# AleoNet/snarkVM

Measured on AMD Instinct MI355X. Metric: BLS12-377 G1 MSM scalar-point pairs/sec (+ Fr NTT elements/sec in ntt_*), higher is better.
Workload: dtype u32 limbs (29-bit radix) modular integer arithmetic, Fq 377-bit / Fr 253-bit; 1 GPU; G1 Pippenger MSM 2^24 (BASELINE.json configs[1]), bases (i+1)G registered in HBM, uniform scalars in HBM; independent instance per GPU; scalars=uniform, lg_ntt=24, window_bits=auto, base_tables=12, table_bits=22, pipelined_batch=True

## Files before the change

### snarkvm_amd/csrc/api_g2.hip

```cpp
#include "msm_batch.hip.h"
#include "serde.hip.h"

static void tu_set_kernel_attributes() {
    HIP_TRY(hipFuncSetAttribute((const void*)scan_one_block_kernel, hipFuncAttributeMaxDynamicSharedMemorySize, (int)(SCAN_ONE_MAX * 4)));
}

struct snarkvm_hip_bases_g2 : bases_handle_t<fq2_t> {};

extern "C" {

RustError snarkvm_hip_msm_g2(void* out, const void* points, size_t npoints, const void* scalars, size_t ffi_affine_sz) {
    API_TRY
#ifdef SV_NO_G2
    throw hip_failure{hipErrorNotSupported, "this development build was compiled without G2 (SV_NO_G2)", __LINE__};
#else
    if (!out) throw hip_failure{hipErrorInvalidValue, "msm_g2: null output", __LINE__};
    g_rt.configure();
    if (npoints == 0) {
        write_infinity<fq2_t>(out);
    } else {
        if (!points || !scalars) throw hip_failure{hipErrorInvalidValue, "msm_g2: null argument", __LINE__};
        msm_host_chunked<fq2_t>(out, points, npoints, scalars, ffi_affine_sz);
    }
#endif
    API_CATCH
}

RustError snarkvm_hip_register_bases_g2(snarkvm_hip_bases_g2_t** handle, const void* points, size_t npoints, size_t ffi_affine_sz, int tables,
                                        int window_bits) {
    API_TRY
#ifdef SV_NO_G2
    throw hip_failure{hipErrorNotSupported, "this development build was compiled without G2 (SV_NO_G2)", __LINE__};
#else
    if (!handle || (npoints && !points)) throw hip_failure{hipErrorInvalidValue, "register_bases_g2: null argument", __LINE__};
    if (ffi_affine_sz < 200 || (ffi_affine_sz & 7)) throw hip_failure{hipErrorInvalidValue, "register_bases_g2: bad stride", __LINE__};
    check_tables(tables, window_bits, "register_bases_g2");
    const int nd = g_rt.ndev();
    std::unique_ptr<snarkvm_hip_bases_g2> h(new snarkvm_hip_bases_g2());
    h->n = npoints;
    h->tables = tables;
    h->table_bits = window_bits ? window_bits : 256 / tables;
    h->d.assign(nd, nullptr);
    if (npoints) {
        try {
            std::vector<int> all;
            for (int d = 0; d < nd; d++) all.push_back(d);
            for_each_device(all, [&](int dev) {
                lane_guard lg(dev);
                lane_t& c = lg.c();
                HIP_TRY(hipMalloc((void**)&h->d[dev], (size_t)tables * npoints * sizeof(aff_mem_t<fq2_t>)));
                c.bases_tmp.ensure(npoints * ffi_affine_sz);
                HIP_TRY(hipMemcpyAsync(c.bases_tmp.p, points, npoints * ffi_affine_sz, hipMemcpyHostToDevice, c.stream));
                convert_bases<fq2_t>(c, c.bases_tmp.as<uint8_t>(), ffi_affine_sz, npoints, h->d[dev]);
                precompute_tables_run<fq2_t>(c, h->d[dev], npoints, tables, h->table_bits);
                bases_to_lazy_form(c, h->d[dev], (size_t)tables * npoints);
                HIP_TRY(hipStreamSynchronize(c.stream));
            });
        } catch (...) {
            h->free_all();
            throw;
        }
    }
    *handle = h.release();
#endif
    API_CATCH
}
void snarkvm_hip_free_bases_g2(snarkvm_hip_bases_g2_t* h) {
    if (!h) return;
    h->free_all();
    delete h;
}
#ifndef SV_NO_G2
static RustError msm_g2_single_coalesced(void* out, const snarkvm_hip_bases_g2_t* h, size_t offset, size_t npoints, const void* scalars, int scalars_on_device,
                                         int window_bits) {
    API_TRY
    if (scalars_on_device && g_rt.device_of(scalars) < 0)
        throw hip_failure{hipErrorInvalidValue, "device pointer does not belong to a device in use (snarkvm_hip_set_devices)", __LINE__};
    msm_ticket_t t;
    t.req.off0 = offset, t.req.n0 = npoints, t.req.scalars = scalars, t.req.out = out;
    t.on_device = scalars_on_device ? 1 : 0;
    t.window_bits = window_bits;
    msm_coalesced<fq2_t>(*h, &t, 1);
    API_CATCH
}
static RustError msm_g2_scope_enqueue(void* out, const snarkvm_hip_bases_g2_t* h, size_t offset, size_t npoints, const void* scalars, int window_bits, bool* queued) {
    API_TRY
    msm_req_t one;
    one.off0 = offset, one.n0 = npoints, one.scalars = scalars, one.out = out;
    *queued = msm_scope_enqueue<fq2_t>(*h, &one, 1, 1, 0, window_bits);
    API_CATCH
}
#endif
RustError snarkvm_hip_msm_g2_registered(void* out, const snarkvm_hip_bases_g2_t* h, size_t offset, size_t npoints, const void* scalars,
                                        int scalars_on_device, int window_bits) {
#ifndef SV_NO_G2
    if (h && out && scalars && offset + npoints <= h->n && (!window_bits || (window_bits >= 2 && window_bits <= MSM_C_MAX)) && g_rt.configured) {
        if (tl_scope().lane && (tl_scope().flags & SNARKVM_HIP_SCOPE_ASYNC_MSM) && scalars_on_device && npoints) {
            bool queued = false;
            const RustError e = msm_g2_scope_enqueue(out, h, offset, npoints, scalars, window_bits, &queued);
            if (e.code || queued) return e;
        }
        if (msm_coalescible(*h, npoints, window_bits)) return msm_g2_single_coalesced(out, h, offset, npoints, scalars, scalars_on_device, window_bits);
    }
#endif
    API_BEGIN_DEV(device_for(scalars, (scalars_on_device && npoints) ? 1 : 0))
#ifdef SV_NO_G2
    throw hip_failure{hipErrorNotSupported, "this development build was compiled without G2 (SV_NO_G2)", __LINE__};
#else
    if (!h || offset + npoints > h->n) throw hip_failure{hipErrorInvalidValue, "msm_g2_registered: range exceeds the registered bases", __LINE__};
    if (window_bits && (window_bits < 2 || window_bits > MSM_C_MAX)) throw hip_failure{hipErrorInvalidValue, "msm_g2_registered: window_bits must be 0 or 2..23", __LINE__};
    if (!out || (npoints && !scalars)) throw hip_failure{hipErrorInvalidValue, "msm_g2_registered: null argument", __LINE__};
    const uint4* d_sc = (const uint4*)scalars;
    if (!scalars_on_device && npoints) {
        c.scalars_tmp.ensure(npoints * 32);
        c.phase_begin("msm_h2d");
        HIP_TRY(hipMemcpyAsync(c.scalars_tmp.p, scalars, npoints * 32, hipMemcpyHostToDevice, c.stream));
        c.phase_end();
        d_sc = c.scalars_tmp.as<uint4>();
    }
    msm_req_t one;
    one.off0 = offset, one.n0 = npoints;
    msm_job_t<fq2_t> job = msm_handle_job<fq2_t>(*h, c.dev->logical, one);
    job.scalars = d_sc;
    job.window_bits = window_bits;
    msm_run_sync<fq2_t>(c, job, out);
#endif
    API_END
}
RustError snarkvm_hip_msm_g2_registered_batch(void* outs, const snarkvm_hip_bases_g2_t* h, size_t count, const size_t* offsets, const size_t* npoints,
                                              const void* const* scalars, int scalars_on_device, int window_bits) {
    API_TRY
#ifdef SV_NO_G2
    throw hip_failure{hipErrorNotSupported, "this development build was compiled without G2 (SV_NO_G2)", __LINE__};
#else
    if (!h) throw hip_failure{hipErrorInvalidValue, "msm_g2_registered_batch: null handle", __LINE__};
    if (window_bits && (window_bits < 2 || window_bits > MSM_C_MAX)) throw hip_failure{hipErrorInvalidValue, "msm_g2_registered_batch: window_bits must be 0 or 2..23", __LINE__};
    if (count && (!outs || !offsets || !npoints || !scalars)) throw hip_failure{hipErrorInvalidValue, "msm_g2_registered_batch: null argument", __LINE__};
    std::vector<msm_req_t> req = msm_requests<fq2_t>(outs, count, offsets, npoints, nullptr, nullptr, scalars);
    msm_batch_dispatch<fq2_t>(*h, req, scalars_on_device, 0, window_bits);
#endif
    API_CATCH
}

static RustError g2_deserialize_impl(void* out_affine, const void* bytes, size_t n, int compressed, int validate) {
    API_BEGIN
#ifdef SV_NO_G2
    throw hip_failure{hipErrorNotSupported, "this development build was compiled without G2 (SV_NO_G2)", __LINE__};
#else
    if (n) {
        if (!out_affine || !bytes) throw hip_failure{hipErrorInvalidValue, "g2_deserialize: null argument", __LINE__};
        const size_t psz = compressed ? 96 : 192;
        c.bases_tmp.ensure(n * psz);
        c.poly[0].ensure(n * 200);
        c.serde_status.ensure(4);
        HIP_TRY(hipMemcpyAsync(c.bases_tmp.p, bytes, n * psz, hipMemcpyHostToDevice, c.stream));
        HIP_TRY(hipMemsetAsync(c.serde_status.p, 0, 4, c.stream));
        hipLaunchKernelGGL(g2_deserialize_kernel, dim3((unsigned)((n + 63) / 64)), dim3(64), 0, c.stream, c.bases_tmp.as<uint8_t>(), n, compressed, validate,
                           c.poly[0].as<uint8_t>(), c.serde_status.as<uint32_t>());
        HIP_TRY(hipGetLastError());
        uint32_t st = 0;
        HIP_TRY(hipMemcpyAsync(&st, c.serde_status.p, 4, hipMemcpyDeviceToHost, c.stream));
        HIP_TRY(hipMemcpyAsync(out_affine, c.poly[0].p, n * 200, hipMemcpyDeviceToHost, c.stream));
        HIP_TRY(hipStreamSynchronize(c.stream));
        serde_throw_on_status(st, "g2_deserialize");
    }
#endif
    API_END
}
static RustError g2_serialize_impl(void* out_bytes, const void* affine, size_t n, size_t ffi_affine_sz, int compressed) {
    API_BEGIN
#ifdef SV_NO_G2
    throw hip_failure{hipErrorNotSupported, "this development build was compiled without G2 (SV_NO_G2)", __LINE__};
#else
    if (n) {
        if (!out_bytes || !affine) throw hip_failure{hipErrorInvalidValue, "g2_serialize: null argument", __LINE__};
        if (ffi_affine_sz < 200 || (ffi_affine_sz & 7)) throw hip_failure{hipErrorInvalidValue, "g2_serialize: bad stride", __LINE__};
        c.bases_tmp.ensure(n * ffi_affine_sz);
        const size_t psz = compressed ? 96 : 192;
        c.poly[0].ensure(n * psz);
        HIP_TRY(hipMemcpyAsync(c.bases_tmp.p, affine, n * ffi_affine_sz, hipMemcpyHostToDevice, c.stream));
        hipLaunchKernelGGL(g2_serialize_kernel, dim3((unsigned)((n + 63) / 64)), dim3(64), 0, c.stream, c.bases_tmp.as<uint8_t>(), ffi_affine_sz, n,
                           compressed, c.poly[0].as<uint8_t>());
        HIP_TRY(hipGetLastError());
        HIP_TRY(hipMemcpyAsync(out_bytes, c.poly[0].p, n * psz, hipMemcpyDeviceToHost, c.stream));
        HIP_TRY(hipStreamSynchronize(c.stream));
    }
#endif
    API_END
}

RustError snarkvm_hip_g2_deserialize(void* out_affine, const void* bytes, size_t n, int validate) { return g2_deserialize_impl(out_affine, bytes, n, 0, validate); }
RustError snarkvm_hip_g2_deserialize_compressed(void* out_affine, const void* bytes, size_t n, int validate) {
    return g2_deserialize_impl(out_affine, bytes, n, 1, validate);
}
RustError snarkvm_hip_g2_serialize(void* out_bytes, const void* affine, size_t n, size_t ffi_affine_sz) { return g2_serialize_impl(out_bytes, affine, n, ffi_affine_sz, 0); }
RustError snarkvm_hip_g2_serialize_compressed(void* out_bytes, const void* affine, size_t n, size_t ffi_affine_sz) {
    return g2_serialize_impl(out_bytes, affine, n, ffi_affine_sz, 1);
}

int snarkvm_hip_selftest_fq2_pair(const void* points, size_t npoints, uint64_t seed, int iters) {
#ifdef SV_NO_G2
    (void)points, (void)npoints, (void)seed, (void)iters;
    return -1;
#else
    if (!points || npoints < 2) return -2;
    std::vector<aff_t<fq2_t>> pool;
    for (size_t i = 0; i < npoints; i++) {
        const uint32_t* src = (const uint32_t*)((const uint8_t*)points + 200 * i);
        pool.push_back({fq2_t::from_raw_words(src), fq2_t::from_raw_words(src + 24)});
    }
    auto next = [&]() {
        seed += 0x9E3779B97F4A7C15ull;
        uint64_t z = seed;
        z = (z ^ (z >> 30)) * 0xBF58476D1CE4E5B9ull;
        z = (z ^ (z >> 27)) * 0x94D049BB133111EBull;
        return z ^ (z >> 31);
    };
    auto same = [](const fql_t (&l)[2], const fq2_t& e) { return l[0].to_exact() == e.c0 && l[1].to_exact() == e.c1; };
    xyzz_t<fq2_t> exact = xyzz_t<fq2_t>::inf();
    fq2p::xyzz_pair_t<fq2p::xp_host> pr;
    pr.inf = true;
    int prev = -1;
    bool prev_neg = false;
    for (int it = 0; it < iters; it++) {
        const uint64_t r = next();
        int k = (int)(r % npoints);
        bool neg = ((r >> 8) & 1) != 0;
        const int mode = (int)((r >> 16) % 16);
        if (mode == 0 && prev >= 0) k = prev, neg = prev_neg;
        if (mode == 1 && prev >= 0) k = prev, neg = !prev_neg;
        if (mode == 2) {
            exact = xyzz_t<fq2_t>::inf();
            pr.inf = true;
        }
        prev = k;
        prev_neg = neg;
        const aff_t<fq2_t> p = pool[k];
        exact.add_affine(p, neg);
        alignas(128) aff_mem_t<fq2_t> slot;
        const fq_t c406 = fq_t::from_table(FqLConv::C406);
        g2_lazy_slot_t::store(&slot, {p.x.c0 * c406, p.x.c1 * c406}, {p.y.c0 * c406, p.y.c1 * c406}, false);
        fql_t px[2], py[2];
        for (int c = 0; c < 2; c++) ((const g2_lazy_slot_t*)&slot)->component(c, px[c], py[c]);
        pr.madd(px, py, neg);
        if (pr.inf != exact.is_inf()) return it + 1;
        if (!pr.inf && !(same(pr.x, exact.x) && same(pr.y, exact.y) && same(pr.zz, exact.zz) && same(pr.zzz, exact.zzz))) return it + 1;
        if (!pr.inf && (it & 7) == 0) {
            const fql_t* cs[4] = {pr.x, pr.y, pr.zz, pr.zzz};
            const fq2_t* es[4] = {&exact.x, &exact.y, &exact.zz, &exact.zzz};
            for (int c4 = 0; c4 < 4; c4++)
                for (int c = 0; c < 2; c++) {
                    fql_t back;
                    for (int j = 0; j < 13; j++) back.v[j] = cs[c4][c].v[j];
                    if (!(back.to_exact() == (c ? es[c4]->c1 : es[c4]->c0))) return -(it + 1);
                }
        }
    }
    return 0;
#endif
}

RustError snarkvm_hip_devtest_g2_tail_repeat(const void* points, size_t npoints, int m, int hb, int threads, int plane_threads, int hex, int quads, int iters,
                                             uint32_t* report) {
    API_BEGIN
#ifdef SV_NO_G2
    (void)points, (void)npoints, (void)m, (void)hb, (void)threads, (void)plane_threads, (void)hex, (void)quads, (void)iters, (void)report;
    throw hip_failure{hipErrorNotSupported, "this development build was compiled without G2 (SV_NO_G2)", __LINE__};
#else
    if (!points || npoints < 2 || !report || m < 1 || hb < 1 || hb > m || m + hb > 16 || iters < 2 || (threads != 64 && threads != 128 && threads != 256) ||
        (plane_threads != 64 && plane_threads != 128 && plane_threads != 256))
        throw hip_failure{hipErrorInvalidValue, "devtest_g2_tail_repeat: bad arguments", __LINE__};
    typedef xyzz_mem_t<fq2_t> mem_t;
    const uint32_t nb = 1u << (m + hb);
    std::vector<uint32_t> cnt(nb), start(nb);
    uint32_t E = 0;
    for (uint32_t k = 0; k < nb; k++) {
        const uint32_t h = (k * 2654435761u) >> 28;
        cnt[k] = h == 0 ? 2 : h == 1 ? 0 : 1;
        start[k] = E;
        E += cnt[k];
    }
    std::vector<mem_t> sums(E);
    for (uint32_t k = 0; k < nb; k++)
        for (uint32_t q = start[k]; q < start[k] + cnt[k]; q++) {
            const uint32_t q0 = start[k];
            const uint32_t* src = (const uint32_t*)((const uint8_t*)points + 200 * (size_t)((q0 * 7u + 3u) % npoints));
            xyzz_t<fq2_t> a = xyzz_t<fq2_t>::inf();
            a.add_affine({fq2_t::from_raw_words(src), fq2_t::from_raw_words(src + 24)}, ((q0 >> 3) & 1) != 0);
            store_xyzz<fq2_t>(&sums[q], a);
        }
    const size_t nslots = (size_t)1 << (m + 1), nbits = (size_t)m + 1, nplanes = 2 * nbits;
    c.part_a.ensure(E * sizeof(mem_t));
    c.cnt_a.ensure(nb * 4);
    c.start_a.ensure(nb * 4);
    c.fold_sums.ensure(2 * nslots * sizeof(mem_t));
    c.planes.ensure(nplanes * sizeof(mem_t));
    c.tail_flags.ensure((nslots + nplanes) * 4);
    std::vector<uint32_t> flag_copy(nslots + nplanes, 0);
    HIP_TRY(hipMemcpyAsync(c.part_a.p, sums.data(), E * sizeof(mem_t), hipMemcpyHostToDevice, c.stream));
    HIP_TRY(hipMemcpyAsync(c.cnt_a.p, cnt.data(), nb * 4, hipMemcpyHostToDevice, c.stream));
    HIP_TRY(hipMemcpyAsync(c.start_a.p, start.data(), nb * 4, hipMemcpyHostToDevice, c.stream));
    HIP_TRY(hipMemsetAsync(c.fold_sums.p, 0, 2 * nslots * sizeof(mem_t), c.stream));
    HIP_TRY(hipMemsetAsync(c.tail_flags.p, 0, (nslots + nplanes) * 4, c.stream));
    std::vector<uint8_t> first(nslots * sizeof(mem_t)), got(nslots * sizeof(mem_t)), p_first(nplanes * sizeof(mem_t)), p_got(nplanes * sizeof(mem_t));
    for (int i = 0; i < 10; i++) report[i] = 0;
    int nfirst = 0;
    auto same_point = [](const xyzz_t<fq2_t>& a, const xyzz_t<fq2_t>& b) {
        if (a.is_inf() || b.is_inf()) return a.is_inf() == b.is_inf();
        return a.x * b.zz == b.x * a.zz && a.y * b.zzz == b.y * a.zzz;
    };
    for (int it = 0; it < iters; it++) {
        mem_t* out = c.fold_sums.as<mem_t>() + (it ? nslots : 0);
        uint32_t* fold_flags = c.tail_flags.as<uint32_t>();
        uint32_t* plane_flags = fold_flags + nslots;
        const dim3 fold_grid((1u << m) + (1u << hb), 1u), plane_grid((unsigned)nbits, 2u);
        hipLaunchKernelGGL((msm_fold_kernel<fq2_t>), fold_grid, dim3((unsigned)threads), 0, c.stream, (const mem_t*)c.part_a.as<mem_t>(),
                           (const uint32_t*)c.start_a.as<uint32_t>(), (const uint32_t*)c.cnt_a.as<uint32_t>(), out, m, hb, hex, quads & 2 ? 1 : 0, fold_flags);
        hipLaunchKernelGGL((msm_fold_fix_kernel<fq2_t>), fold_grid, dim3(64), 0, c.stream, (const mem_t*)c.part_a.as<mem_t>(), (const uint32_t*)c.start_a.as<uint32_t>(),
                           (const uint32_t*)c.cnt_a.as<uint32_t>(), out, m, hb, (const uint32_t*)fold_flags);
        hipLaunchKernelGGL((msm_bitplane_kernel<fq2_t, true>), plane_grid, dim3((unsigned)plane_threads), 0, c.stream, (const mem_t*)c.fold_sums.as<mem_t>(),
                           (const uint32_t*)nullptr, (const uint32_t*)nullptr, c.planes.as<mem_t>(), nb, m, hb, hex, quads & 1, plane_flags);
        hipLaunchKernelGGL((msm_bitplane_fix_kernel<fq2_t, true>), plane_grid, dim3(64), 0, c.stream, (const mem_t*)c.fold_sums.as<mem_t>(), (const uint32_t*)nullptr,
                           (const uint32_t*)nullptr, c.planes.as<mem_t>(), nb, m, hb, (const uint32_t*)plane_flags);
        if (!it) HIP_TRY(hipMemcpyAsync(flag_copy.data(), fold_flags, (nslots + nplanes) * 4, hipMemcpyDeviceToHost, c.stream));
        HIP_TRY(hipGetLastError());
        HIP_TRY(hipMemcpyAsync(it ? got.data() : first.data(), out, nslots * sizeof(mem_t), hipMemcpyDeviceToHost, c.stream));
        HIP_TRY(hipMemcpyAsync(it ? p_got.data() : p_first.data(), c.planes.p, nplanes * sizeof(mem_t), hipMemcpyDeviceToHost, c.stream));
        HIP_TRY(hipStreamSynchronize(c.stream));
        if (!it) continue;
        uint32_t bad = 0;
        for (size_t sl = 0; sl + 1 < nslots; sl++)
            if (!same_point(load_xyzz<fq2_t>((const mem_t*)&first[sl * sizeof(mem_t)]), load_xyzz<fq2_t>((const mem_t*)&got[sl * sizeof(mem_t)]))) {
                bad++;
                if (nfirst < 4) report[4 + nfirst++] = (uint32_t)sl;
            }
        report[0] += bad ? 1 : 0;
        report[1] += bad;
        bad = 0;
        for (size_t pl = 0; pl < nplanes; pl++)
            if (!same_point(load_xyzz<fq2_t>((const mem_t*)&p_first[pl * sizeof(mem_t)]), load_xyzz<fq2_t>((const mem_t*)&p_got[pl * sizeof(mem_t)]))) bad++;
        report[2] += bad ? 1 : 0;
        report[3] += bad;
    }
    report[8] = report[9] = 0;
    for (size_t sl = 0; sl + 1 < nslots; sl++) report[8] += flag_copy[sl] ? 1 : 0;
    for (size_t pl = 0; pl < nplanes; pl++) report[9] += flag_copy[nslots + pl] ? 1 : 0;
#endif
    API_END
}

int snarkvm_hip_selftest_g2_hex(const void* points, size_t npoints, uint64_t seed, int iters) {
#ifdef SV_NO_G2
    (void)points, (void)npoints, (void)seed, (void)iters;
    return -1;
#else
    if (!points || npoints < 2) return -2;
    std::vector<aff_t<fq2_t>> pool;
    for (size_t i = 0; i < npoints; i++) {
        const uint32_t* src = (const uint32_t*)((const uint8_t*)points + 200 * i);
        pool.push_back({fq2_t::from_raw_words(src), fq2_t::from_raw_words(src + 24)});
    }
    auto next = [&]() {
        seed += 0x9E3779B97F4A7C15ull;
        uint64_t z = seed;
        z = (z ^ (z >> 30)) * 0xBF58476D1CE4E5B9ull;
        z = (z ^ (z >> 27)) * 0x94D049BB133111EBull;
        return z ^ (z >> 31);
    };
    auto partial = [&](int terms) {
        xyzz_t<fq2_t> a = xyzz_t<fq2_t>::inf();
        for (int t = 0; t < terms; t++) {
            const uint64_t r = next();
            a.add_affine(pool[r % npoints], ((r >> 40) & 1) != 0);
        }
        return a;
    };
    for (int it = 0; it < iters; it++) {
        const int mode = (int)(next() % 12);
        xyzz_t<fq2_t> a = partial(1 + (int)(next() % 3)), b = partial(1 + (int)(next() % 3));
        if (mode == 0) b = a;
        if (mode == 1) b = a, b.y = b.y.neg();
        if (mode == 2) a = xyzz_t<fq2_t>::inf();
        if (mode == 3) b = xyzz_t<fq2_t>::inf();
        if (mode == 4) a = xyzz_t<fq2_t>::inf(), b = xyzz_t<fq2_t>::inf();
        xyzz_t<fq2_t> want = a;
        want.add(b);
        if (hex_add_host_check(a, b, want)) return it + 1;
        xyzz_t<fq2_t> f = a;
        bool flagged = false;
        f.add_flag(b, flagged);
        const bool same_x = !a.is_inf() && !b.is_inf() && a.x * b.zz == b.x * a.zz;
        if (flagged != same_x) return 100000 + it + 1;
        const xyzz_t<fq2_t>& expect = flagged ? a : want;
        if (!(f.x == expect.x && f.y == expect.y && f.zz == expect.zz && f.zzz == expect.zzz)) return 200000 + it + 1;
    }
    return 0;
#endif
}

}
```

### snarkvm_amd/csrc/api_tailtest.hip

```cpp
#include "msm_run.hip.h"

static void tu_set_kernel_attributes() {}

namespace {

enum { TT_REDUCE = 0, TT_MERGE, TT_FOLD, TT_SPARSE };
struct tt_geom_t {
    int m, hb, W, nb, S2, L, slot, fold_threads, plane_threads, hex, quads, run_fix;
};
struct tt_args_t {
    int stage;
    tt_geom_t g;
    const uint8_t* points;
    size_t npoints;
    const int32_t* terms;
    const uint64_t* seeds;
    size_t nentries;
    const uint32_t *start, *cnt;
    size_t nbt;
    uint32_t *out, *status, *flags;
    size_t nout;
    uint32_t* aux;
};
[[noreturn]] void tt_bad(const char* what, int line) { throw hip_failure{hipErrorInvalidValue, what, line}; }

template <class E>
E tt_scale(uint64_t seed);
template <>
fq_t tt_scale<fq_t>(uint64_t seed) {
    fq_t l = fq_t::zero();
    for (int i = 0; i < 12; i++) {
        seed += 0x9E3779B97F4A7C15ull;
        uint64_t z = seed;
        z = (z ^ (z >> 30)) * 0xBF58476D1CE4E5B9ull;
        z = (z ^ (z >> 27)) * 0x94D049BB133111EBull;
        l.v[i] = (uint32_t)((z ^ (z >> 31)) & LIMB_MASK);
    }
    l.v[0] |= 1;
    return l;
}
template <>
fq2_t tt_scale<fq2_t>(uint64_t seed) {
    return {tt_scale<fq_t>(seed), tt_scale<fq_t>(~seed)};
}
template <class T, class E>
void tt_put(xyzz_mem_t<T>* dst, const xyzz_t<E>& a) {
    if (a.is_inf()) {
        memset(dst, 0, sizeof *dst);
        return;
    }
    if constexpr (std::is_same<T, fqz_t>::value)
        store_xyzz<fqz_t>(dst, xyzz_t<fqz_t>{{fql_t::from_exact(a.x)}, {fql_t::from_exact(a.y)}, {fql_t::from_exact(a.zz)}, {fql_t::from_exact(a.zzz)}});
    else
        store_xyzz<T>(dst, a);
}
template <class T, class E>
xyzz_t<E> tt_get(const xyzz_mem_t<T>* src) {
    const xyzz_t<T> p = load_xyzz<T>(src);
    if constexpr (std::is_same<T, fqz_t>::value) {
        if (p.is_inf()) return xyzz_t<E>::inf();
        return {p.x.to_exact(), p.y.to_exact(), p.zz.to_exact(), p.zzz.to_exact()};
    } else {
        return p;
    }
}
bool tt_is_fill(const void* p, size_t bytes) {
    for (size_t i = 0; i < bytes; i++)
        if (((const uint8_t*)p)[i] != 0xff) return false;
    return true;
}
int tt_log2(uint32_t v) {
    int l = 0;
    while ((1u << l) < v) l++;
    return l;
}

template <class T, class E, size_t STRIDE>
void tt_run(lane_t& c, const tt_args_t& a) {
    typedef xyzz_mem_t<T> mem_t;
    constexpr bool G2 = std::is_same<E, fq2_t>::value;
    constexpr size_t CW = sizeof(typename E::mem_t) / 4;
    const tt_geom_t& g = a.g;
    const size_t nbt = a.nbt, nacc = a.stage == TT_MERGE ? nbt * (size_t)g.L : 0, nent = a.nentries + nacc;
    hipStream_t st = c.stream;
    std::vector<aff_t<E>> pool(a.npoints);
    for (size_t i = 0; i < a.npoints; i++) {
        const uint32_t* src = (const uint32_t*)(a.points + STRIDE * i);
        pool[i] = {E::from_raw_words(src), E::from_raw_words(src + CW)};
        if (pool[i].is_inf()) tt_bad("devtest_msm_tail: a pool point at infinity", __LINE__);
    }
    std::vector<mem_t> ent(nent ? nent : 1);
    for (size_t e = 0; e < nent; e++) {
        xyzz_t<E> p = xyzz_t<E>::inf();
        for (int j = 0; j < 3; j++) {
            const int32_t t = a.terms[3 * e + j];
            if (!t) continue;
            const size_t idx = (size_t)(t < 0 ? -(int64_t)t : (int64_t)t) - 1;
            if (idx >= a.npoints) tt_bad("devtest_msm_tail: a term outside the pool", __LINE__);
            p.add_affine(pool[idx], t < 0);
        }
        if (a.seeds[e] && !p.is_inf()) {
            const E l = tt_scale<E>(a.seeds[e]), l2 = l.sqr(), l3 = l2 * l;
            p = {p.x * l2, p.y * l3, p.zz * l2, p.zzz * l3};
        }
        tt_put<T, E>(&ent[e], p);
    }
    c.part_a.ensure((a.nentries + 1) * sizeof(mem_t));
    c.start_a.ensure((nbt + 1) * 4);
    c.cnt_a.ensure((nbt + 1) * 4);
    if (a.nentries) HIP_TRY(hipMemcpyAsync(c.part_a.p, ent.data(), a.nentries * sizeof(mem_t), hipMemcpyHostToDevice, st));
    HIP_TRY(hipMemcpyAsync(c.start_a.p, a.start, (nbt + 1) * 4, hipMemcpyHostToDevice, st));
    HIP_TRY(hipMemcpyAsync(c.cnt_a.p, a.cnt, nbt * 4, hipMemcpyHostToDevice, st));
    HIP_TRY(hipMemsetAsync(c.cnt_a.as<uint32_t>() + nbt, 0, 4, st));
    const mem_t* sums = c.part_a.as<mem_t>();
    const uint32_t *start = c.start_a.as<uint32_t>(), *cnt = c.cnt_a.as<uint32_t>();
    std::vector<mem_t> got(a.nout);
    std::vector<uint32_t> flag_copy(a.nout, 0);
    if (a.stage == TT_REDUCE) {
        c.cnt_b.ensure((nbt + 1) * 4);
        c.start_b.ensure((nbt + 1) * 4);
        c.scan_tmp.ensure(scan_tmp_elems(nbt + 1) * 4);
        c.part_b.ensure(a.nout * sizeof(mem_t));
        HIP_TRY(hipMemsetAsync(c.part_b.p, 0xff, a.nout * sizeof(mem_t), st));
        HIP_TRY(hipMemsetAsync(c.start_b.p, 0xff, (nbt + 1) * 4, st));
        hipLaunchKernelGGL(msm_alloc_kernel, dim3((unsigned)((nbt + 1 + 255) / 256)), dim3(256), 0, st, cnt, c.cnt_b.as<uint32_t>(), (uint32_t)nbt, (uint32_t)g.S2);
        exclusive_scan_u32(st, c.cnt_b.as<uint32_t>(), c.start_b.as<uint32_t>(), nbt + 1, c.scan_tmp.as<uint32_t>());
        hipLaunchKernelGGL((msm_reduce_kernel<T>), dim3((unsigned)((a.nout + 255) / 256)), dim3(256), 0, st, sums, start, cnt, (const uint32_t*)c.start_b.as<uint32_t>(),
                           c.part_b.as<mem_t>(), (uint32_t)nbt, (uint32_t)g.S2);
        HIP_TRY(hipGetLastError());
        HIP_TRY(hipMemcpyAsync(a.aux, c.start_b.p, (nbt + 1) * 4, hipMemcpyDeviceToHost, st));
        HIP_TRY(hipMemcpyAsync(got.data(), c.part_b.p, a.nout * sizeof(mem_t), hipMemcpyDeviceToHost, st));
    } else if (a.stage == TT_MERGE) {
        c.part_b.ensure(nacc * sizeof(mem_t));
        HIP_TRY(hipMemcpyAsync(c.part_b.p, ent.data() + a.nentries, nacc * sizeof(mem_t), hipMemcpyHostToDevice, st));
        hipLaunchKernelGGL((msm_bucket_merge_kernel<T>), dim3((unsigned)((nbt + 255) / 256)), dim3(256), 0, st, sums, start, cnt, c.part_b.as<mem_t>(), (uint32_t)nbt,
                           (uint32_t)g.L, (uint32_t)g.slot);
        HIP_TRY(hipGetLastError());
        HIP_TRY(hipMemcpyAsync(got.data(), c.part_b.p, nacc * sizeof(mem_t), hipMemcpyDeviceToHost, st));
    } else {
        const bool fold = a.stage == TT_FOLD;
        const int nbits = fold ? g.m + 1 : tt_log2((uint32_t)g.nb) + 1;
        const size_t nslots = fold ? (size_t)g.W << (g.m + 1) : 0, nplanes = (size_t)(fold ? 2 * g.W : g.W) * nbits;
        c.fold_sums.ensure((nslots + 1) * sizeof(mem_t));
        c.planes.ensure(nplanes * sizeof(mem_t));
        c.tail_flags.ensure((nslots + nplanes) * 4);
        HIP_TRY(hipMemsetAsync(c.fold_sums.p, 0xff, (nslots + 1) * sizeof(mem_t), st));
        HIP_TRY(hipMemsetAsync(c.planes.p, 0xff, nplanes * sizeof(mem_t), st));
        HIP_TRY(hipMemsetAsync(c.tail_flags.p, 0xff, (nslots + nplanes) * 4, st));
        uint32_t* fold_flags = G2 ? c.tail_flags.as<uint32_t>() : nullptr;
        uint32_t* plane_flags = G2 ? fold_flags + nslots : nullptr;
        mem_t* fs = c.fold_sums.as<mem_t>();
        mem_t* planes = c.planes.as<mem_t>();
        const dim3 plane_grid((unsigned)nbits, (unsigned)(fold ? 2 * g.W : g.W));
        if (fold) {
            const dim3 fold_grid((1u << g.m) + (1u << g.hb), (unsigned)g.W);
            hipLaunchKernelGGL((msm_fold_kernel<T>), fold_grid, dim3((unsigned)g.fold_threads), 0, st, sums, start, cnt, fs, g.m, g.hb, g.hex, (g.quads >> 1) & 1, fold_flags);
            if constexpr (TAIL_FLAGGED<T>::value)
                if (g.run_fix) hipLaunchKernelGGL((msm_fold_fix_kernel<T>), fold_grid, dim3(64), 0, st, sums, start, cnt, fs, g.m, g.hb, (const uint32_t*)fold_flags);
            hipLaunchKernelGGL((msm_bitplane_kernel<T, true>), plane_grid, dim3((unsigned)g.plane_threads), 0, st, (const mem_t*)fs, (const uint32_t*)nullptr,
                               (const uint32_t*)nullptr, planes, (uint32_t)1 << (g.m + g.hb), g.m, g.hb, g.hex, g.quads & 1, plane_flags);
            if constexpr (TAIL_FLAGGED<T>::value)
                if (g.run_fix)
                    hipLaunchKernelGGL((msm_bitplane_fix_kernel<T, true>), plane_grid, dim3(64), 0, st, (const mem_t*)fs, (const uint32_t*)nullptr, (const uint32_t*)nullptr,
                                       planes, (uint32_t)1 << (g.m + g.hb), g.m, g.hb, (const uint32_t*)plane_flags);
        } else {
            hipLaunchKernelGGL((msm_bitplane_kernel<T, false>), plane_grid, dim3((unsigned)g.plane_threads), 0, st, sums, start, cnt, planes, (uint32_t)g.nb, 0, 0, g.hex, 0,
                               plane_flags);
            if constexpr (TAIL_FLAGGED<T>::value)
                if (g.run_fix)
                    hipLaunchKernelGGL((msm_bitplane_fix_kernel<T, false>), plane_grid, dim3(64), 0, st, sums, start, cnt, planes, (uint32_t)g.nb, 0, 0, (const uint32_t*)plane_flags);
        }
        HIP_TRY(hipGetLastError());
        if (nslots) HIP_TRY(hipMemcpyAsync(got.data(), fs, nslots * sizeof(mem_t), hipMemcpyDeviceToHost, st));
        HIP_TRY(hipMemcpyAsync(got.data() + nslots, planes, nplanes * sizeof(mem_t), hipMemcpyDeviceToHost, st));
        if (G2) HIP_TRY(hipMemcpyAsync(flag_copy.data(), c.tail_flags.p, (nslots + nplanes) * 4, hipMemcpyDeviceToHost, st));
    }
    HIP_TRY(hipStreamSynchronize(st));
    for (size_t i = 0; i < a.nout; i++) {
        uint32_t* dst = a.out + 3 * CW * i;
        a.flags[i] = flag_copy[i];
        if (a.stage != TT_MERGE && tt_is_fill(&got[i], sizeof(mem_t))) {
            a.status[i] = 1;
            memset(dst, 0xff, 3 * CW * 4);
            continue;
        }
        a.status[i] = (a.stage == TT_MERGE && memcmp(&got[i], &ent[a.nentries + i], sizeof(mem_t)) == 0) ? 2u : 0u;
        const jac_t<E> j = tt_get<T, E>(&got[i]).to_jacobian();
        j.x.to_raw_words(dst);
        j.y.to_raw_words(dst + CW);
        j.z.to_raw_words(dst + 2 * CW);
    }
}

}

extern "C" {

RustError snarkvm_hip_devtest_msm_tail(int arith, int stage, const int32_t* geom, const void* points, size_t npoints, const int32_t* terms, const uint64_t* seeds,
                                       size_t nentries, const uint32_t* start, const uint32_t* cnt, size_t nbt, void* out, uint32_t* status, uint32_t* flags, size_t nout,
                                       uint32_t* aux) {
    API_BEGIN
    if (arith < 0 || arith > 2 || stage < TT_REDUCE || stage > TT_SPARSE) tt_bad("devtest_msm_tail: arith must be 0 .. 2, stage 0 .. 3", __LINE__);
#ifdef SV_NO_G2
    if (arith == 2) throw hip_failure{hipErrorNotSupported, "this development build was compiled without G2 (SV_NO_G2)", __LINE__};
#endif
    if (!geom || !points || !terms || !seeds || !start || !cnt || !out || !status || !flags || (stage == TT_REDUCE && !aux))
        tt_bad("devtest_msm_tail: null argument", __LINE__);
    tt_args_t a;
    a.stage = stage;
    a.g = {geom[0], geom[1], geom[2], geom[3], geom[4], geom[5], geom[6], geom[7], geom[8], geom[9], geom[10], geom[11]};
    const tt_geom_t& g = a.g;
    auto threads_ok = [](int t) { return t == 64 || t == 128 || t == 256; };
    if (npoints == 0 || npoints > 4096 || nbt == 0 || nbt > ((size_t)1 << 17) || nentries > ((size_t)1 << 20)) tt_bad("devtest_msm_tail: sizes out of range", __LINE__);
    if ((g.hex != 0 && g.hex != 1) || g.quads < 0 || g.quads > 3 || (g.run_fix != 0 && g.run_fix != 1) || (arith != 2 && (g.hex || g.run_fix)))
        tt_bad("devtest_msm_tail: hex, quads or run_fix out of range (hex and run_fix are G2 switches)", __LINE__);
    size_t want_out = 0;
    bool contiguous = false;
    if (stage == TT_REDUCE) {
        if (g.S2 < 2 || g.S2 > 64) tt_bad("devtest_msm_tail: S2 must be 2 .. 64", __LINE__);
        size_t T = 0;
        for (size_t k = 0; k < nbt; k++) T += ((size_t)cnt[k] + g.S2 - 1) / g.S2;
        if (nout < T || nout > T + 4096 || nout == 0) tt_bad("devtest_msm_tail: nout must cover the round's partial sums (and at most 4096 more)", __LINE__);
        want_out = nout;
    } else if (stage == TT_MERGE) {
        if (g.L < 1 || g.L > 8 || g.slot < 0 || g.slot >= g.L) tt_bad("devtest_msm_tail: L must be 1 .. 8, slot < L", __LINE__);
        want_out = nbt * (size_t)g.L;
    } else if (stage == TT_FOLD) {
        if (g.m < 1 || g.hb < 1 || g.hb > g.m || g.hb > 11 || g.m > 11 || g.W < 1 || g.W > 64) tt_bad("devtest_msm_tail: fold geometry out of range (1 <= hb <= m <= 11)", __LINE__);
        if (!threads_ok(g.fold_threads) || !threads_ok(g.plane_threads)) tt_bad("devtest_msm_tail: threads must be 64, 128 or 256", __LINE__);
        if (((g.quads & 2) && g.fold_threads == 64) || ((g.quads & 1) && g.plane_threads == 64)) tt_bad("devtest_msm_tail: no quad-strided loop with 64 threads", __LINE__);
        if (nbt != ((size_t)g.W << (g.m + g.hb))) tt_bad("devtest_msm_tail: nbt must be W * 2^(m + hb)", __LINE__);
        want_out = ((size_t)g.W << (g.m + 1)) + 2 * (size_t)g.W * (g.m + 1);
        contiguous = true;
    } else {
        if (g.nb < 2 || g.nb > 1024 || (g.nb & (g.nb - 1)) || g.W < 1 || g.W > 64) tt_bad("devtest_msm_tail: nb must be a power of two, 2 .. 1024", __LINE__);
        if (!threads_ok(g.plane_threads) || g.quads) tt_bad("devtest_msm_tail: threads must be 64, 128 or 256, and the unfolded planes have no quad-strided loop", __LINE__);
        if (nbt != (size_t)g.W * g.nb) tt_bad("devtest_msm_tail: nbt must be W * nb", __LINE__);
        int nbits = 1;
        while ((1 << (nbits - 1)) < g.nb) nbits++;
        want_out = (size_t)g.W * nbits;
        contiguous = true;
    }
    if (nout != want_out) tt_bad("devtest_msm_tail: nout does not match the stage's outputs", __LINE__);
    for (size_t k = 0; k < nbt; k++) {
        if ((size_t)start[k] + cnt[k] > nentries) tt_bad("devtest_msm_tail: a list overruns the entries", __LINE__);
        if (contiguous && start[k + 1] != start[k] + cnt[k]) tt_bad("devtest_msm_tail: the fold and the bit planes walk lists laid out bucket after bucket", __LINE__);
    }
    if (contiguous && (start[0] != 0 || start[nbt] != nentries)) tt_bad("devtest_msm_tail: the lists must cover the entries", __LINE__);
    a.points = (const uint8_t*)points;
    a.npoints = npoints;
    a.terms = terms;
    a.seeds = seeds;
    a.nentries = nentries;
    a.start = start;
    a.cnt = cnt;
    a.nbt = nbt;
    a.out = (uint32_t*)out;
    a.status = status;
    a.flags = flags;
    a.nout = nout;
    a.aux = aux;
    if (arith == 0) tt_run<fq_t, fq_t, 104>(c, a);
    if (arith == 1) tt_run<fqz_t, fq_t, 104>(c, a);
#ifndef SV_NO_G2
    if (arith == 2) tt_run<fq2_t, fq2_t, 200>(c, a);
#endif
    API_END
}

}
```

### snarkvm_amd/csrc/msm.hip.h

```cpp
#pragma once
#include <stdlib.h>

#include <type_traits>

#include "ec.hip.h"
#include "ffl.hip.h"
#include "ffl2.hip.h"
#include "hex2.hip.h"
#include "tuning.hip.h"

namespace sv {

struct msm_plan_t {
    size_t n;
    int c;
    int W;
    int J;
    int Wd;
    uint32_t nb;
    uint32_t nbt;
    uint32_t chunk;
    uint32_t nchunks;
    uint32_t S, S2;
    uint32_t L;
    int rounds;
    uint32_t bias[10];
};

static inline int msm_pick_c(size_t n) {
    if (n > ((size_t)1 << 17)) return 16;
    int lg = 0;
    while (((size_t)1 << lg) < n) lg++;
    int c = lg - 4;
    if (c < 2) c = 2;
    if (c > 11) c = 11;
    return c;
}
static constexpr int MSM_C_MAX = 23;
static constexpr int MSM_BIAS_BITS = 288;
static inline msm_plan_t msm_make_plan(size_t n, int c_override = 0, int tables = 1, int table_bits = 0) {
    msm_plan_t p;
    p.n = n;
    p.J = tables < 1 ? 1 : tables;
    if (p.J == 1) {
        p.c = c_override ? c_override : msm_pick_c(n);
        if (p.c > 16) p.c = 16;
        p.W = (254 + p.c - 1) / p.c;
    } else {
        const int part = table_bits > 0 ? table_bits : 256 / p.J;
        if (c_override) {
            p.c = c_override;
            if (p.c > part) p.c = part;
            while (part % p.c) p.c--;
            if (p.c > 16 && p.c != part) {
                p.c = 16;
                while (part % p.c) p.c--;
            }
            if (p.c < 2) p.c = part <= 16 ? part : 2;
        } else if (part <= 16) {
            p.c = n >= 4096 ? 16 : 8;
            if (p.c > part) p.c = part;
            while (part % p.c) p.c--;
            if (p.c < 2) p.c = part;
        } else {
            double best = 0;
            p.c = 0;
            for (int d = 2; d <= part && d <= MSM_C_MAX; d++) {
                if (part % d || (d > 16 && d != part)) continue;
                const double cost = (double)p.J * (part / d) * (double)n + (double)(part / d) * (double)((size_t)1 << (d - 1)) * 8.0;
                if (p.c == 0 || cost < best) {
                    best = cost;
                    p.c = d;
                }
            }
            if (p.c == 0) p.c = 1;
        }
        p.W = part / p.c;
    }
    p.Wd = p.W * p.J;
    p.nb = 1u << (p.c - 1);
    p.nbt = (uint32_t)p.W * p.nb;
    p.chunk = (1u << 18) / (uint32_t)p.J;
    p.chunk &= ~7u;
    if (p.chunk > n) p.chunk = (uint32_t)(n ? n : 1);
    p.nchunks = (uint32_t)((n + p.chunk - 1) / p.chunk);
    const int env_S = tuning().seg, env_S2 = tuning().seg2, env_L = tuning().fold_l;
    {
        const size_t E = (size_t)p.Wd * n;
        const size_t smax = E >= ((size_t)1 << 27) ? 128 : 64, round = (size_t)1 << 16;
        const size_t k = (E + smax * round - 1) / (smax * round);
        const size_t sfill = k ? (E + k * round - 1) / (k * round) : 4;
        p.S = (uint32_t)(sfill < 4 ? 4 : sfill);
    }
    if (env_S > 0) p.S = env_S;
    p.S2 = env_S2 > 1 ? env_S2 : 16;
    p.L = env_L > 0 ? (uint32_t)env_L : 8;
    if (p.L > p.nb) p.L = p.nb;
    while (p.nb % p.L) p.L--;
    p.rounds = 0;
    size_t m = ((size_t)p.J * n + p.S - 1) / p.S;
    while (m > 1) {
        m = (m + p.S2 - 1) / p.S2;
        p.rounds++;
    }
    for (int i = 0; i < 10; i++) p.bias[i] = 0;
    for (int w = 0; w < p.Wd; w++) {
        int bit = p.c - 1 + p.c * w;
        if (bit >= MSM_BIAS_BITS) break;
        p.bias[bit / 32] |= 1u << (bit % 32);
    }
    return p;
}

static constexpr int SCAN_TILE = 2048;
static __global__ void scan_tile_kernel(const uint32_t* in, uint32_t* out, uint32_t* block_sums, size_t n) {
    __shared__ uint32_t sh[256];
    const size_t base = (size_t)blockIdx.x * SCAN_TILE + (size_t)threadIdx.x * 8;
    uint32_t v[8], s = 0;
#pragma unroll
    for (int i = 0; i < 8; i++) {
        v[i] = (base + i < n) ? in[base + i] : 0u;
        s += v[i];
    }
    sh[threadIdx.x] = s;
    __syncthreads();
    for (int off = 1; off < 256; off <<= 1) {
        uint32_t t = (threadIdx.x >= (unsigned)off) ? sh[threadIdx.x - off] : 0u;
        __syncthreads();
        sh[threadIdx.x] += t;
        __syncthreads();
    }
    uint32_t run = sh[threadIdx.x] - s;
#pragma unroll
    for (int i = 0; i < 8; i++) {
        if (base + i < n) out[base + i] = run;
        run += v[i];
    }
    if (threadIdx.x == 255 && block_sums) block_sums[blockIdx.x] = sh[255];
}
static __global__ void scan_add_kernel(uint32_t* out, const uint32_t* block_offsets, size_t n) {
    const size_t base = (size_t)blockIdx.x * SCAN_TILE + (size_t)threadIdx.x * 8;
    const uint32_t add = block_offsets[blockIdx.x];
#pragma unroll
    for (int i = 0; i < 8; i++)
        if (base + i < n) out[base + i] += add;
}
static inline size_t scan_tmp_elems(size_t n) {
    size_t tot = 0;
    while (n > 1) {
        n = (n + SCAN_TILE - 1) / SCAN_TILE;
        tot += n + 1;
        if (n == 1) break;
    }
    return tot + 8;
}
static constexpr uint32_t SCAN_ONE_THREADS = 1024, SCAN_ONE_MAX = 33 * SCAN_ONE_THREADS;
static __global__ void __launch_bounds__(1024) scan_one_block_kernel(const uint32_t* in, uint32_t* out, uint32_t n, uint32_t per) {
    extern __shared__ uint32_t scan_sm[];
    __shared__ uint32_t wave_tot[16];
    const uint32_t t = threadIdx.x;
    for (uint32_t i = t; i < n; i += SCAN_ONE_THREADS) scan_sm[i] = in[i];
    __syncthreads();
    const uint32_t lo = t * per, hi = lo + per < n ? lo + per : n;
    uint32_t sum = 0;
    for (uint32_t i = lo; i < hi; i++) sum += scan_sm[i];
    uint32_t incl = sum;
    for (int off = 1; off < 64; off <<= 1) {
        const uint32_t u = (uint32_t)__shfl_up((int)incl, off);
        if ((t & 63) >= (uint32_t)off) incl += u;
    }
    if ((t & 63) == 63) wave_tot[t >> 6] = incl;
    __syncthreads();
    uint32_t base = 0;
    for (uint32_t w = 0; w < (t >> 6); w++) base += wave_tot[w];
    uint32_t run = base + incl - sum;
    for (uint32_t i = lo; i < hi; i++) {
        const uint32_t v = scan_sm[i];
        scan_sm[i] = run;
        run += v;
    }
    __syncthreads();
    for (uint32_t i = t; i < n; i += SCAN_ONE_THREADS) out[i] = scan_sm[i];
}
static inline void exclusive_scan_u32(hipStream_t st, const uint32_t* in, uint32_t* out, size_t n, uint32_t* tmp) {
    if (n == 0) return;
    const int one_launch = tuning().scan1;
    if (one_launch && n > (size_t)SCAN_TILE && n <= (size_t)SCAN_ONE_MAX) {
        const uint32_t per = (uint32_t)((n + SCAN_ONE_THREADS - 1) / SCAN_ONE_THREADS) | 1u;
        hipLaunchKernelGGL(scan_one_block_kernel, dim3(1), dim3(SCAN_ONE_THREADS), (size_t)n * 4, st, in, out, (uint32_t)n, per);
        return;
    }
    const size_t blocks = (n + SCAN_TILE - 1) / SCAN_TILE;
    hipLaunchKernelGGL(scan_tile_kernel, dim3((unsigned)blocks), dim3(256), 0, st, in, out, tmp, n);
    if (blocks > 1) {
        exclusive_scan_u32(st, tmp, tmp, blocks, tmp + blocks + 1);
        hipLaunchKernelGGL(scan_add_kernel, dim3((unsigned)blocks), dim3(256), 0, st, out, tmp, n);
    }
}

template <class F>
SV_HD void store_base_slot(aff_mem_t<F>* slot, const uint32_t* xw, const uint32_t* yw, bool inf, int form406) {
    aff_t<F> a = aff_t<F>::inf();
    if (!inf) {
        a.x = F::from_raw_words(xw);
        a.y = F::from_raw_words(yw);
    }
    store_aff<F>(slot, a);
}
template <>
SV_HD void store_base_slot<fq_t>(aff_mem_t<fq_t>* slot, const uint32_t* xw, const uint32_t* yw, bool inf, int form406) {
    if (form406) {
        const fq_t c = fq_t::from_table(FqLConv::C399);
        g1_lazy_slot_t::store(slot, fq_t::unpack(xw) * c, fq_t::unpack(yw) * c, inf);
        return;
    }
    g1_aff_t a = g1_aff_t::inf();
    if (!inf) {
        a.x = fq_t::from_raw_words(xw);
        a.y = fq_t::from_raw_words(yw);
    }
    store_aff<fq_t>(slot, a);
}
template <>
SV_HD void store_base_slot<fq2_t>(aff_mem_t<fq2_t>* slot, const uint32_t* xw, const uint32_t* yw, bool inf, int form406) {
    if (form406) {
        const fq_t c = fq_t::from_table(FqLConv::C399);
        g2_lazy_slot_t::store(slot, {fq_t::unpack(xw) * c, fq_t::unpack(xw + 12) * c}, {fq_t::unpack(yw) * c, fq_t::unpack(yw + 12) * c}, inf);
        return;
    }
    aff_t<fq2_t> a = aff_t<fq2_t>::inf();
    if (!inf) {
        a.x = fq2_t::from_raw_words(xw);
        a.y = fq2_t::from_raw_words(yw);
    }
    store_aff<fq2_t>(slot, a);
}
static __global__ void g2_bases_to_form406_kernel(aff_mem_t<fq2_t>* slots, size_t n) {
    const size_t i = blockIdx.x * (size_t)blockDim.x + threadIdx.x;
    if (i >= n) return;
    const fq_t c = fq_t::from_table(FqLConv::C406);
    const aff_t<fq2_t> a = load_aff<fq2_t>(&slots[i]);
    g2_lazy_slot_t::store(&slots[i], {a.x.c0 * c, a.x.c1 * c}, {a.y.c0 * c, a.y.c1 * c}, a.is_inf());
}
static __global__ void g1_bases_to_form406_kernel(g1_aff_mem_t* slots, size_t n) {
    const size_t i = blockIdx.x * (size_t)blockDim.x + threadIdx.x;
    if (i >= n) return;
    const fq_t c = fq_t::from_table(FqLConv::C406);
    const g1_aff_t a = g1_load_aff(&slots[i]);
    g1_lazy_slot_t::store(&slots[i], a.x * c, a.y * c, a.is_inf());
}
template <class F>
__global__ void convert_bases_kernel(const uint8_t* in, size_t stride, size_t n, aff_mem_t<F>* out, int form406) {
    size_t i = blockIdx.x * (size_t)blockDim.x + threadIdx.x;
    if (i >= n) return;
    const uint32_t* src = (const uint32_t*)(in + i * stride);
    constexpr int MW = F::MEM_WORDS;
    uint32_t xw[MW], yw[MW];
#pragma unroll
    for (int k = 0; k < MW; k++) {
        xw[k] = src[k];
        yw[k] = src[MW + k];
    }
    const uint32_t inf = src[2 * MW] & 0xffu;
    store_base_slot<F>(&out[i], xw, yw, inf != 0, form406);
}

struct msm_digit_params_t {
    uint32_t bias[10];
    int c, W;
    size_t n;
    int montgomery;
};
template <class DT>
__global__ void __launch_bounds__(256) msm_digits_kernel(const uint4* __restrict__ scalars, DT* __restrict__ digits,
                                                         msm_digit_params_t p) {
    __shared__ uint4 stage[512];
    const size_t nblk = (p.n + 255) / 256;
    for (size_t blk = blockIdx.x; blk < nblk; blk += gridDim.x) {
        const size_t first = blk * 256;
        const size_t cnt = (p.n - first < 256) ? (p.n - first) : 256;
        for (int k = threadIdx.x; k < 512; k += 256)
            if ((size_t)(k >> 1) < cnt) stage[k] = scalars[first * 2 + k];
        __syncthreads();
        if (threadIdx.x < cnt) {
            const uint4 lo = stage[2 * threadIdx.x], hi = stage[2 * threadIdx.x + 1];
            uint32_t s[11] = {lo.x, lo.y, lo.z, lo.w, hi.x, hi.y, hi.z, hi.w, 0u, 0u, 0u};
            if (p.montgomery) {
                fr_t c32 = fr_t::zero();
                c32.v[0] = 32;
                (fr_t::unpack(s) * c32).pack(s);
            }
            uint64_t carry = 0;
#pragma unroll
            for (int k = 0; k < 10; k++) {
                carry += (uint64_t)s[k] + p.bias[k];
                s[k] = (uint32_t)carry;
                carry >>= 32;
            }
            const uint32_t mask = (1u << p.c) - 1;
            const size_t i = first + threadIdx.x;
            for (int w = 0; w < p.W; w++) {
                const int bit = p.c * w, wi = bit >> 5, sh = bit & 31;
                uint64_t two = (uint64_t)s[wi] | ((uint64_t)s[wi + 1] << 32);
                digits[(size_t)w * p.n + i] = (DT)((uint32_t)(two >> sh) & mask);
            }
        }
        __syncthreads();
    }
}

static __global__ void msm_alloc_kernel(const uint32_t* cnt_in, uint32_t* cnt_out, uint32_t nbt, uint32_t S) {
    uint32_t k = blockIdx.x * blockDim.x + threadIdx.x;
    if (k > nbt) return;
    cnt_out[k] = (k == nbt) ? 0u : (cnt_in[k] + S - 1) / S;
}
__device__ __forceinline__ uint32_t find_bucket(const uint32_t* start, uint32_t nbt, uint32_t t) {
    uint32_t lo = 0, hi = nbt;
    while (hi - lo > 1) {
        const uint32_t mid = (lo + hi) >> 1;
        if (start[mid] <= t)
            lo = mid;
        else
            hi = mid;
    }
    return lo;
}
template <class F>
__global__ void __launch_bounds__(256) msm_reduce_kernel(const xyzz_mem_t<F>* __restrict__ in,
                                                         const uint32_t* __restrict__ in_start,
                                                         const uint32_t* __restrict__ in_cnt,
                                                         const uint32_t* __restrict__ out_start,
                                                         xyzz_mem_t<F>* __restrict__ out, uint32_t nbt, uint32_t S2) {
    const uint32_t t = blockIdx.x * blockDim.x + threadIdx.x;
    if (t >= out_start[nbt]) return;
    const uint32_t k = find_bucket(out_start, nbt, t);
    const uint32_t j = t - out_start[k];
    const uint32_t lo = in_start[k] + j * S2;
    uint32_t hi = lo + S2;
    const uint32_t end = in_start[k] + in_cnt[k];
    if (hi > end) hi = end;
    xyzz_t<F> acc = load_xyzz<F>(&in[lo]);
    for (uint32_t pos = lo + 1; pos < hi; pos++) acc.add(load_xyzz<F>(&in[pos]));
    store_xyzz<F>(&out[t], acc);
}

template <class F>
__global__ void __launch_bounds__(256) msm_bucket_merge_kernel(const xyzz_mem_t<F>* __restrict__ part, const uint32_t* __restrict__ start,
                                                               const uint32_t* __restrict__ cnt, xyzz_mem_t<F>* __restrict__ acc, uint32_t nbt, uint32_t L,
                                                               uint32_t slot) {
    const uint32_t k = blockIdx.x * blockDim.x + threadIdx.x;
    if (k >= nbt) return;
    const uint32_t c = cnt[k];
    if (!c) return;
    const uint32_t lo = start[k];
    xyzz_mem_t<F>* dst = &acc[(size_t)k * L + slot];
    xyzz_t<F> a = load_xyzz<F>(dst);
    for (uint32_t i = 0; i < c; i++) a.add(load_xyzz<F>(&part[lo + i]));
    store_xyzz<F>(dst, a);
}
static __global__ void msm_sink_lists_kernel(uint32_t* __restrict__ start, uint32_t* __restrict__ cnt, uint32_t nbt, uint32_t L) {
    const uint32_t k = blockIdx.x * blockDim.x + threadIdx.x;
    if (k > nbt) return;
    start[k] = k * L;
    cnt[k] = k < nbt ? L : 0u;
}

__device__ __forceinline__ fq_t shfl_xor_field(const fq_t& a, int mask) {
    fq_t r;
#pragma unroll
    for (int i = 0; i < fq_t::N; i++) r.v[i] = (uint32_t)__shfl_xor((int)a.v[i], mask);
    return r;
}
__device__ __forceinline__ fq2_t shfl_xor_field(const fq2_t& a, int mask) { return {shfl_xor_field(a.c0, mask), shfl_xor_field(a.c1, mask)}; }
__device__ __forceinline__ fqz_t shfl_xor_field(const fqz_t& a, int mask) {
    fqz_t r;
#pragma unroll
    for (int i = 0; i < fqz_t::N; i++) r.a.v[i] = __shfl_xor(a.a.v[i], mask);
    SV_OPAQUE_13(r.a.v);
    return r;
}
template <class F>
__device__ __forceinline__ xyzz_t<F> shfl_xor_point(const xyzz_t<F>& a, int mask) {
    return {shfl_xor_field(a.x, mask), shfl_xor_field(a.y, mask), shfl_xor_field(a.zz, mask), shfl_xor_field(a.zzz, mask)};
}
template <int CTRL>
__device__ __forceinline__ fq_t quad_perm_field(const fq_t& a) {
    fq_t r;
#pragma unroll
    for (int i = 0; i < fq_t::N; i++) r.v[i] = (uint32_t)__builtin_amdgcn_mov_dpp((int)a.v[i], CTRL, 0xf, 0xf, true);
    return r;
}
template <int CTRL>
__device__ __forceinline__ fq2_t quad_perm_field(const fq2_t& a) {
    return {quad_perm_field<CTRL>(a.c0), quad_perm_field<CTRL>(a.c1)};
}
template <int CTRL>
__device__ __forceinline__ fqz_t quad_perm_field(const fqz_t& a) {
    fqz_t r;
#pragma unroll
    for (int i = 0; i < fqz_t::N; i++) r.a.v[i] = __builtin_amdgcn_mov_dpp(a.a.v[i], CTRL, 0xf, 0xf, true);
    SV_OPAQUE_13(r.a.v);
    return r;
}
template <int L, class F>
__device__ __forceinline__ F quad_bcast(const F& a) {
    return quad_perm_field<L * 0x55>(a);
}
__device__ __forceinline__ fq_t select_field(bool c, const fq_t& a, const fq_t& b) {
    fq_t r;
#pragma unroll
    for (int i = 0; i < fq_t::N; i++) r.v[i] = c ? a.v[i] : b.v[i];
    return r;
}
__device__ __forceinline__ fq2_t select_field(bool c, const fq2_t& a, const fq2_t& b) {
    return {select_field(c, a.c0, b.c0), select_field(c, a.c1, b.c1)};
}
__device__ __forceinline__ fqz_t select_field(bool c, const fqz_t& a, const fqz_t& b) {
    fqz_t r;
#pragma unroll
    for (int i = 0; i < fqz_t::N; i++) r.a.v[i] = c ? a.a.v[i] : b.a.v[i];
    return r;
}
template <class F>
__device__ __forceinline__ xyzz_t<F> select_point(bool c, const xyzz_t<F>& a, const xyzz_t<F>& b) {
    return {select_field(c, a.x, b.x), select_field(c, a.y, b.y), select_field(c, a.zz, b.zz), select_field(c, a.zzz, b.zzz)};
}

template <class F>
struct TAIL_FLAGGED {
    static constexpr bool value = sizeof(F) > 64;
};
template <class F>
__device__ __forceinline__ void tail_add(xyzz_t<F>& acc, const xyzz_t<F>& o, bool& dbl) {
    if constexpr (TAIL_FLAGGED<F>::value)
        acc.add_flag(o, dbl);
    else
        acc.add(o);
}
template <class F>
__device__ __forceinline__ void quad_add(xyzz_t<F>& acc, const xyzz_t<F>& o, bool& dbl) {
    const uint32_t r = threadIdx.x & 3;
    const bool inf1 = acc.is_inf(), inf2 = o.is_inf();
    F a = select_field(r < 2, select_field(r == 0, acc.x, o.x), select_field(r == 2, acc.y, o.y));
    F b = select_field(r < 2, select_field(r == 0, o.zz, acc.zz), select_field(r == 2, o.zzz, acc.zzz));
    const F m1 = a * b;
    const F t = quad_perm_field<0xB1>(m1);
    const F d = select_field((r & 1) != 0, m1, t) - select_field((r & 1) != 0, t, m1);
    const bool same_x = !inf1 && !inf2 && r < 2 && d.is_zero();
    if (__ballot(same_x) != 0) {
        if constexpr (TAIL_FLAGGED<F>::value)
            dbl = true;
        else
            acc.add(o);
        return;
    }
    a = select_field((r & 1) == 0, d, select_field(r == 1, acc.zz, acc.zzz));
    b = select_field((r & 1) == 0, d, select_field(r == 1, o.zz, o.zzz));
    const F m2 = a * b;
    const F pp = quad_bcast<0>(m2);
    a = select_field(r == 1, t, select_field(r == 2, quad_bcast<1>(m2), d));
    const F m3 = a * pp;
    const F ppp = quad_bcast<0>(m3), q = quad_bcast<1>(m3);
    const F x3 = m2 - ppp - q.dbl();
    a = select_field(r == 0, quad_bcast<3>(m2), select_field(r == 2, d, t));
    b = select_field(r == 2, q - x3, ppp);
    const F m4 = a * b;
    xyzz_t<F> res;
    res.x = quad_bcast<2>(x3);
    res.y = quad_bcast<2>(m4) - quad_bcast<3>(m4);
    res.zz = quad_bcast<2>(m3);
    res.zzz = quad_bcast<0>(m4);
    acc = select_point(inf2, acc, select_point(inf1, o, res));
}
template <class F>
__device__ __forceinline__ void quad_add(xyzz_t<F>& acc, const xyzz_t<F>& o) {
    static_assert(!TAIL_FLAGGED<F>::value, "the Fq2 form reports P + P instead of computing it");
    bool unused = false;
    quad_add(acc, o, unused);
}
template <class F>
__device__ __forceinline__ void block_sum(xyzz_t<F>& acc, xyzz_mem_t<F>* sh, int hex, bool from_quads, bool& dbl) {
    if (!from_quads) {
        const xyzz_t<F> o = shfl_xor_point(acc, 1);
        const bool odd = (threadIdx.x & 1) != 0;
        xyzz_t<F> lo = select_point(odd, o, acc);
        tail_add(lo, select_point(odd, acc, o), dbl);
        acc = lo;
    }
    if (!from_quads) {
        const xyzz_t<F> o = shfl_xor_point(acc, 2);
        const bool hi = (threadIdx.x & 2) != 0;
        xyzz_t<F> lo = select_point(hi, o, acc);
        quad_add(lo, select_point(hi, acc, o), dbl);
        acc = lo;
    }
    if constexpr (std::is_same<F, fq2_t>::value) {
        if (hex) {
            {
                const xyzz_t<F> o = shfl_xor_point(acc, 4);
                const bool hi = (threadIdx.x & 4) != 0;
                xyzz_t<F> lo = select_point(hi, o, acc);
                quad_add(lo, select_point(hi, acc, o), dbl);
                acc = lo;
            }
#pragma unroll 1
            for (int off = 8; off < 64; off <<= 1) {
                const xyzz_t<F> o = shfl_xor_point(acc, off);
                const bool hi = (threadIdx.x & off) != 0;
                xyzz_t<F> lo = select_point(hi, o, acc);
                hex_add(lo, select_point(hi, acc, o), dbl);
                acc = lo;
            }
            if (blockDim.x == 64) return;
            const uint32_t wv = threadIdx.x >> 6, nw = blockDim.x >> 6;
            if ((threadIdx.x & 63) == 0) store_xyzz<F>(&sh[wv], acc);
            __syncthreads();
            if (threadIdx.x < 64) {
                const uint32_t pair = (threadIdx.x >> 4) & (nw / 2 - 1);
                acc = load_xyzz<F>(&sh[2 * pair]);
                hex_add(acc, load_xyzz<F>(&sh[2 * pair + 1]), dbl);
#pragma unroll 1
                for (uint32_t off = 16; off < 8 * nw; off <<= 1) {
                    const xyzz_t<F> o = shfl_xor_point(acc, (int)off);
                    const bool hi = (threadIdx.x & off) != 0;
                    xyzz_t<F> lo = select_point(hi, o, acc);
                    hex_add(lo, select_point(hi, acc, o), dbl);
                    acc = lo;
                }
            }
            return;
        }
    }
#pragma unroll 1
    for (int off = 4; off < 64; off <<= 1) quad_add(acc, shfl_xor_point(acc, off), dbl);
    if (blockDim.x == 64) return;
    const uint32_t wv = threadIdx.x >> 6, nw = blockDim.x >> 6;
    if ((threadIdx.x & 63) == 0) store_xyzz<F>(&sh[wv], acc);
    __syncthreads();
    if (threadIdx.x < 64) {
        const uint32_t pair = (threadIdx.x >> 2) & (nw / 2 - 1);
        acc = load_xyzz<F>(&sh[2 * pair]);
        quad_add(acc, load_xyzz<F>(&sh[2 * pair + 1]), dbl);
#pragma unroll 1
        for (uint32_t off = 4; off < 2 * nw; off <<= 1) quad_add(acc, shfl_xor_point(acc, (int)off), dbl);
    }
}
template <class F>
__device__ __forceinline__ void tail_store(xyzz_mem_t<F>* out, uint32_t* flags, size_t slot, const xyzz_t<F>& acc, bool dbl) {
    if constexpr (TAIL_FLAGGED<F>::value) {
        const int any = __syncthreads_or(dbl ? 1 : 0);
        if (threadIdx.x == 0) flags[slot] = (uint32_t)any;
    }
    if (threadIdx.x == 0) store_xyzz<F>(&out[slot], acc);
}
template <class F>
struct TAIL_WAVES {
    static constexpr int value = sizeof(F) <= 64 ? 2 : 1;
};
__device__ __forceinline__ void block_running_sums(uint32_t* s, uint32_t n, uint32_t* tmp) {
    const uint32_t B = blockDim.x, t = threadIdx.x;
    const uint32_t per = (n + B - 1) / B;
    const uint32_t lo = 1 + t * per, hi = lo + per < n + 1 ? lo + per : n + 1;
    uint32_t sum = 0;
    for (uint32_t i = lo; i < hi; i++) sum += s[i];
    tmp[t] = sum;
    __syncthreads();
    if (t < 64) {
        const uint32_t e = B >> 6;
        uint32_t v[4], own = 0;
        for (uint32_t q = 0; q < e; q++) {
            v[q] = tmp[t * e + q];
            own += v[q];
        }
        uint32_t incl = own;
        for (int off = 1; off < 64; off <<= 1) {
            const uint32_t u = (uint32_t)__shfl_up((int)incl, off);
            if (t >= (uint32_t)off) incl += u;
        }
        uint32_t run = incl - own;
        for (uint32_t q = 0; q < e; q++) {
            tmp[t * e + q] = run;
            run += v[q];
        }
    }
    __syncthreads();
    uint32_t run = tmp[t];
    for (uint32_t i = lo; i < hi; i++) {
        run += s[i];
        s[i] = run;
    }
    __syncthreads();
}
__device__ __forceinline__ uint32_t find_segment(const uint32_t* off, uint32_t nseg, uint32_t p) {
    uint32_t lo = 0, hi = nseg;
    while (hi - lo > 1) {
        const uint32_t mid = (lo + hi) >> 1;
        if (off[mid] <= p) lo = mid; else hi = mid;
    }
    return lo;
}
static constexpr uint32_t TAIL_MAX_SEG = 2048;
template <class F>
__global__ void __launch_bounds__(256, TAIL_WAVES<F>::value) msm_fold_kernel(const xyzz_mem_t<F>* __restrict__ sums, const uint32_t* __restrict__ start,
                                                       const uint32_t* __restrict__ cnt, xyzz_mem_t<F>* __restrict__ out, int m, int hb, int hex, int quads,
                                                       uint32_t* __restrict__ flags) {
    __shared__ xyzz_mem_t<F> sh[16];
    __shared__ uint32_t s_off[TAIL_MAX_SEG + 1], s_start[TAIL_MAX_SEG], s_tmp[256];
    const uint32_t nlo = 1u << m, nhi = 1u << hb;
    const uint32_t w = blockIdx.y;
    const uint32_t kbase = w << (m + hb);
    const bool column = blockIdx.x >= nhi;
    const uint32_t fixed = column ? blockIdx.x - nhi : blockIdx.x;
    if (!column && fixed == 0) return;
    const size_t slot = ((size_t)w << (m + 1)) + (column ? fixed : nlo + fixed - 1);
    bool dbl = false;
    uint32_t nseg;
    if (column) {
        for (uint32_t i = threadIdx.x; i < nhi; i += blockDim.x) {
            const uint32_t k = kbase + (i << m) + fixed;
            s_start[i] = start[k];
            s_off[i + 1] = cnt[k];
        }
        if (threadIdx.x == 0) s_off[0] = 0;
        __syncthreads();
        block_running_sums(s_off, nhi, s_tmp);
        nseg = nhi;
    } else {
        const uint32_t k0 = kbase + (fixed << m);
        if (threadIdx.x == 0) {
            s_start[0] = start[k0];
            s_off[0] = 0;
            s_off[1] = start[k0 + nlo - 1] + cnt[k0 + nlo - 1] - start[k0];
        }
        __syncthreads();
        nseg = 1;
    }
    const uint32_t total = s_off[nseg];
    xyzz_t<F> acc = xyzz_t<F>::inf();
    if (quads) {
        const uint32_t nq = blockDim.x >> 2, qid = threadIdx.x >> 2;
        const uint32_t iters = (total + nq - 1) / nq;
#pragma unroll 1
        for (uint32_t it = 0; it < iters; it++) {
            const uint32_t p = qid + it * nq;
            xyzz_t<F> x = xyzz_t<F>::inf();
            if (p < total) {
                const uint32_t i = find_segment(s_off, nseg, p);
                x = load_xyzz<F>(&sums[s_start[i] + (p - s_off[i])]);
            }
            if (it == 0)
                acc = x;
            else
                quad_add(acc, x, dbl);
        }
        block_sum<F>(acc, sh, hex, true, dbl);
    } else {
        for (uint32_t p = threadIdx.x; p < total; p += blockDim.x) {
            const uint32_t i = find_segment(s_off, nseg, p);
            tail_add(acc, load_xyzz<F>(&sums[s_start[i] + (p - s_off[i])]), dbl);
        }
        block_sum<F>(acc, sh, hex, false, dbl);
    }
    tail_store<F>(out, flags, slot, acc, dbl);
}
template <class F>
__global__ void __launch_bounds__(64) msm_fold_fix_kernel(const xyzz_mem_t<F>* __restrict__ sums, const uint32_t* __restrict__ start, const uint32_t* __restrict__ cnt,
                                                          xyzz_mem_t<F>* __restrict__ out, int m, int hb, const uint32_t* __restrict__ flags) {
    const uint32_t nlo = 1u << m, nhi = 1u << hb;
    const uint32_t w = blockIdx.y;
    const uint32_t kbase = w << (m + hb);
    const bool column = blockIdx.x >= nhi;
    const uint32_t fixed = column ? blockIdx.x - nhi : blockIdx.x;
    if (!column && fixed == 0) return;
    const size_t slot = ((size_t)w << (m + 1)) + (column ? fixed : nlo + fixed - 1);
    if (!flags[slot]) return;
    xyzz_t<F> acc = xyzz_t<F>::inf();
    const uint32_t k0 = kbase + (fixed << m);
    const uint32_t nouter = column ? nhi : 1u;
    for (uint32_t i = column ? threadIdx.x : 0u; i < nouter; i += column ? 64u : 1u) {
        const uint32_t k = kbase + (i << m) + fixed;
        const uint32_t q0 = column ? start[k] : start[k0] + threadIdx.x;
        const uint32_t q1 = column ? q0 + cnt[k] : start[k0 + nlo - 1] + cnt[k0 + nlo - 1];
#pragma unroll 1
        for (uint32_t q = q0; q < q1; q += column ? 1u : 64u) acc.add_inlined_dbl(load_xyzz<F>(&sums[q]));
    }
#pragma unroll 1
    for (int off = 1; off < 64; off <<= 1) acc.add_inlined_dbl(shfl_xor_point(acc, off));
    if (threadIdx.x == 0) store_xyzz<F>(&out[slot], acc);
}
template <class F, bool DENSE>
__global__ void __launch_bounds__(256, TAIL_WAVES<F>::value) msm_bitplane_kernel(const xyzz_mem_t<F>* __restrict__ sums, const uint32_t* __restrict__ start,
                                                           const uint32_t* __restrict__ cnt, xyzz_mem_t<F>* __restrict__ planes, uint32_t nb,
                                                           int m, int hb, int hex, int quads, uint32_t* __restrict__ flags) {
    __shared__ xyzz_mem_t<F> sh[16];
    __shared__ uint32_t s_off[DENSE ? 1 : TAIL_MAX_SEG + 1];
    const uint32_t j = blockIdx.x, tw = blockIdx.y, nbits = gridDim.x;
    const size_t slot = (size_t)tw * nbits + j;
    xyzz_t<F> acc = xyzz_t<F>::inf();
    bool dbl = false;
    if (DENSE) {
        const uint32_t w = tw >> 1, sub = tw & 1;
        const uint32_t N = sub ? (1u << hb) - 1 : (1u << m);
        const size_t base = ((size_t)w << (m + 1)) + ((size_t)sub << m);
        if (quads) {
            const uint32_t nq = blockDim.x >> 2, qid = threadIdx.x >> 2;
            const uint32_t iters = (N + nq - 1) / nq;
#pragma unroll 1
            for (uint32_t it = 0; it < iters; it++) {
                const uint32_t i = qid + it * nq;
                xyzz_t<F> x = xyzz_t<F>::inf();
                if (i < N && (((i + 1) >> j) & 1)) x = load_xyzz<F>(&sums[base + i]);
                if (it == 0)
                    acc = x;
                else
                    quad_add(acc, x, dbl);
            }
            block_sum<F>(acc, sh, hex, true, dbl);
            tail_store<F>(planes, flags, slot, acc, dbl);
            return;
        }
        for (uint32_t i = threadIdx.x; i < N; i += blockDim.x)
            if (((i + 1) >> j) & 1) tail_add(acc, load_xyzz<F>(&sums[base + i]), dbl);
    } else {
        const size_t base = (size_t)tw * nb;
        const uint32_t p0 = start[base];
        for (uint32_t i = threadIdx.x; i < nb; i += blockDim.x) s_off[i] = start[base + i] - p0;
        if (threadIdx.x == 0) s_off[nb] = start[base + nb - 1] + cnt[base + nb - 1] - p0;
        __syncthreads();
        const uint32_t total = s_off[nb];
        for (uint32_t p = threadIdx.x; p < total; p += blockDim.x) {
            const uint32_t i = find_segment(s_off, nb, p);
            if (((i + 1) >> j) & 1) tail_add(acc, load_xyzz<F>(&sums[p0 + p]), dbl);
        }
    }
    block_sum<F>(acc, sh, hex, false, dbl);
    tail_store<F>(planes, flags, slot, acc, dbl);
}
template <class F, bool DENSE>
__global__ void __launch_bounds__(64) msm_bitplane_fix_kernel(const xyzz_mem_t<F>* __restrict__ sums, const uint32_t* __restrict__ start, const uint32_t* __restrict__ cnt,
                                                              xyzz_mem_t<F>* __restrict__ planes, uint32_t nb, int m, int hb, const uint32_t* __restrict__ flags) {
    __shared__ uint32_t s_off[DENSE ? 1 : TAIL_MAX_SEG + 1];
    const uint32_t j = blockIdx.x, tw = blockIdx.y, nbits = gridDim.x;
    const size_t slot = (size_t)tw * nbits + j;
    if (!flags[slot]) return;
    xyzz_t<F> acc = xyzz_t<F>::inf();
    size_t first;
    uint32_t total;
    if (DENSE) {
        const uint32_t w = tw >> 1, sub = tw & 1;
        total = sub ? (1u << hb) - 1 : (1u << m);
        first = ((size_t)w << (m + 1)) + ((size_t)sub << m);
    } else {
        const size_t base = (size_t)tw * nb;
        const uint32_t p0 = start[base];
        for (uint32_t i = threadIdx.x; i < nb; i += 64u) s_off[i] = start[base + i] - p0;
        if (threadIdx.x == 0) s_off[nb] = start[base + nb - 1] + cnt[base + nb - 1] - p0;
        __syncthreads();
        total = s_off[nb];
        first = p0;
    }
#pragma unroll 1
    for (uint32_t p = threadIdx.x; p < total; p += 64u) {
        const uint32_t i = DENSE ? p : find_segment(s_off, nb, p);
        if (((i + 1) >> j) & 1) acc.add_inlined_dbl(load_xyzz<F>(&sums[first + p]));
    }
#pragma unroll 1
    for (int off = 1; off < 64; off <<= 1) acc.add_inlined_dbl(shfl_xor_point(acc, off));
    if (threadIdx.x == 0) store_xyzz<F>(&planes[slot], acc);
}

#define SV_TAIL_FOLD_KERNELS(PREFIX, F)                                                                                                                             \
    PREFIX template __global__ void msm_fold_kernel<F>(const xyzz_mem_t<F>*, const uint32_t*, const uint32_t*, xyzz_mem_t<F>*, int, int, int, int, uint32_t*);
#define SV_TAIL_PLANE_KERNELS(PREFIX, F)                                                                                                                            \
    PREFIX template __global__ void msm_bitplane_kernel<F, true>(const xyzz_mem_t<F>*, const uint32_t*, const uint32_t*, xyzz_mem_t<F>*, uint32_t, int, int, int, int, uint32_t*); \
    PREFIX template __global__ void msm_bitplane_kernel<F, false>(const xyzz_mem_t<F>*, const uint32_t*, const uint32_t*, xyzz_mem_t<F>*, uint32_t, int, int, int, int, uint32_t*);
#define SV_TAIL_KERNELS(PREFIX, F) SV_TAIL_FOLD_KERNELS(PREFIX, F) SV_TAIL_PLANE_KERNELS(PREFIX, F)
#define SV_TAIL_FIX_KERNELS(PREFIX, F)                                                                                                                              \
    PREFIX template __global__ void msm_fold_fix_kernel<F>(const xyzz_mem_t<F>*, const uint32_t*, const uint32_t*, xyzz_mem_t<F>*, int, int, const uint32_t*);          \
    PREFIX template __global__ void msm_bitplane_fix_kernel<F, true>(const xyzz_mem_t<F>*, const uint32_t*, const uint32_t*, xyzz_mem_t<F>*, uint32_t, int, int, const uint32_t*); \
    PREFIX template __global__ void msm_bitplane_fix_kernel<F, false>(const xyzz_mem_t<F>*, const uint32_t*, const uint32_t*, xyzz_mem_t<F>*, uint32_t, int, int, const uint32_t*);
SV_TAIL_KERNELS(extern, fq_t)
SV_TAIL_KERNELS(extern, fqz_t)
SV_TAIL_KERNELS(extern, fq2_t)
SV_TAIL_FIX_KERNELS(extern, fq2_t)

static constexpr int PRE_RUN = 16;
template <class F>
__global__ void __launch_bounds__(256) precompute_table_kernel(const aff_mem_t<F>* __restrict__ prev, aff_mem_t<F>* __restrict__ next,
                                                               size_t n, int shift, int run, typename F::mem_t* __restrict__ scratch) {
    const size_t t = blockIdx.x * (size_t)blockDim.x + threadIdx.x;
    const size_t first = t * (size_t)run;
    if (first >= n) return;
    const size_t cnt = n - first < (size_t)run ? n - first : (size_t)run;
    typename F::mem_t* sx = scratch + 4 * first;
    F prod = F::one();
    for (size_t i = 0; i < cnt; i++) {
        const aff_t<F> p = load_aff<F>(&prev[first + i]);
        jac_t<F> j = {p.x, p.y, p.is_inf() ? F::zero() : F::one()};
        for (int d = 0; d < shift; d++) j = j.dbl();
        if (!j.is_inf()) prod = prod * j.z;
        j.x.store(&sx[4 * i]);
        j.y.store(&sx[4 * i + 1]);
        j.z.store(&sx[4 * i + 2]);
        prod.store(&sx[4 * i + 3]);
    }
    F inv = prod.inverse();
    for (size_t i = cnt; i-- > 0;) {
        const F z = F::load(&sx[4 * i + 2]);
        aff_t<F> q = aff_t<F>::inf();
        if (!z.is_zero()) {
            const F before = i == 0 ? F::one() : F::load(&sx[4 * i - 1]);
            const F zi = inv * before;
            inv = inv * z;
            const F zi2 = zi.sqr();
            q.x = F::load(&sx[4 * i]) * zi2;
            q.y = F::load(&sx[4 * i + 1]) * (zi2 * zi);
        }
        store_aff<F>(&next[first + i], q);
    }
}
static constexpr size_t PRE_SLAB = (size_t)1 << 20;

static __global__ void g1_to_affine_kernel(const uint32_t* in, uint32_t* out, size_t n) {
    size_t i = blockIdx.x * (size_t)blockDim.x + threadIdx.x;
    if (i >= n) return;
    const uint32_t* src = in + 36 * i;
    uint32_t* dst = out + 26 * i;
    const fq_t z = fq_t::from_raw_words(src + 24);
    if (z.is_zero()) {
        for (int k = 0; k < 12; k++) dst[k] = 0;
        fq_t::one().to_raw_words(dst + 12);
        dst[24] = 1;
        dst[25] = 0;
        return;
    }
    const fq_t x = fq_t::from_raw_words(src), y = fq_t::from_raw_words(src + 12);
    const fq_t zi = z.inverse();
    const fq_t zi2 = zi.sqr();
    (x * zi2).to_raw_words(dst);
    (y * (zi2 * zi)).to_raw_words(dst + 12);
    dst[24] = 0;
    dst[25] = 0;
}

static __global__ void __launch_bounds__(64) g1_sum_kernel(const uint32_t* in, size_t n, uint32_t* out) {
    __shared__ g1_xyzz_mem_t part[64];
    g1_xyzz_t acc = g1_xyzz_t::inf();
    for (size_t i = threadIdx.x; i < n; i += 64) {
        const uint32_t* src = in + 36 * i;
        g1_jac_t j = {fq_t::from_raw_words(src), fq_t::from_raw_words(src + 12), fq_t::from_raw_words(src + 24)};
        acc.add(g1_xyzz_t::from_jacobian(j));
    }
    g1_store_xyzz(&part[threadIdx.x], acc);
    __syncthreads();
    for (int s = 32; s > 0; s >>= 1) {
        if ((int)threadIdx.x < s) {
            g1_xyzz_t a = g1_load_xyzz(&part[threadIdx.x]);
            a.add(g1_load_xyzz(&part[threadIdx.x + s]));
            g1_store_xyzz(&part[threadIdx.x], a);
        }
        __syncthreads();
    }
    if (threadIdx.x == 0) {
        const g1_jac_t r = g1_load_xyzz(&part[0]).to_jacobian();
        r.x.to_raw_words(out);
        r.y.to_raw_words(out + 12);
        r.z.to_raw_words(out + 24);
    }
}

static constexpr int GEN_RUN = 32;
static __global__ void __launch_bounds__(256) g1_generate_bases_kernel(g1_aff_mem_t gen, uint64_t start, size_t n, uint8_t* out,
                                                                size_t stride, g1_xyzz_mem_t* scratch_pts,
                                                                fq_mem_t* scratch_prod) {
    const size_t t = blockIdx.x * (size_t)blockDim.x + threadIdx.x;
    const size_t first = t * GEN_RUN;
    if (first >= n) return;
    const size_t cnt = (n - first < (size_t)GEN_RUN) ? (n - first) : (size_t)GEN_RUN;
    const g1_aff_t g = g1_load_aff(&gen);
    const uint64_t k = start + first;
    g1_xyzz_t cur = g1_xyzz_t::inf();
    for (int bit = 63; bit >= 0; bit--) {
        cur = cur.dbl();
        if ((k >> bit) & 1) cur.add_affine(g);
    }
    fq_t prod = fq_t::one();
    for (size_t i = 0; i < cnt; i++) {
        g1_store_xyzz(&scratch_pts[first + i], cur);
        prod = prod * cur.zzz;
        prod.store(&scratch_prod[first + i]);
        cur.add_affine(g);
    }
    fq_t inv = prod.inverse();
    for (size_t i = cnt; i-- > 0;) {
        const g1_xyzz_t pt = g1_load_xyzz(&scratch_pts[first + i]);
        const fq_t zzz_inv = (i == 0) ? inv : inv * fq_t::load(&scratch_prod[first + i - 1]);
        inv = inv * pt.zzz;
        const fq_t zz_inv = zzz_inv.sqr() * pt.zz.sqr();
        uint32_t w[26];
        (pt.x * zz_inv).to_mem_mont().pack(w);
        (pt.y * zzz_inv).to_mem_mont().pack(w + 12);
        w[24] = 0;
        w[25] = 0;
        uint32_t* dst = (uint32_t*)(out + (first + i) * stride);
        for (int q = 0; q < 26; q++) dst[q] = w[q];
    }
}

}
```

### snarkvm_amd/csrc/msm_run.hip.h

```cpp
#pragma once
#include "runtime.hip.h"
#include "ec.hip.h"
#include "msm.hip.h"
#include "msm_sort.hip.h"

static const uint64_t FQ_R[6] = {202099033278250856ull,  5854854902718660529ull, 11492539364873682930ull,
                                 8885205928937022213ull, 5545221690922665192ull, 39800542322357402ull};
template <class F>
static void write_infinity(void* out) {
    const size_t fb = sizeof(typename F::mem_t);
    memset(out, 0, 3 * fb);
    memcpy((uint8_t*)out + fb, FQ_R, 48);
}

static constexpr int MSM_MAX_POS = 320;
template <class F>
struct msm_accum_t {
    xyzz_t<F> at[MSM_MAX_POS];
    bool used[MSM_MAX_POS];
    int top = -1;
    msm_accum_t() {
        for (int i = 0; i < MSM_MAX_POS; i++) used[i] = false;
    }
    void add(int pos, const xyzz_t<F>& p) {
        if (p.is_inf()) return;
        if (pos < 0 || pos >= MSM_MAX_POS) throw std::runtime_error("msm: bit position out of range");
        if (!used[pos]) {
            at[pos] = p;
            used[pos] = true;
        } else {
            at[pos].add(p);
        }
        if (pos > top) top = pos;
    }
    void finish(void* out) const {
        xyzz_t<F> t = xyzz_t<F>::inf();
        for (int p = top; p >= 0; p--) {
            t = t.dbl();
            if (used[p]) t.add(at[p]);
        }
        const jac_t<F> j = t.to_jacobian();
        uint32_t w[3 * F::MEM_WORDS];
        j.x.to_raw_words(w);
        j.y.to_raw_words(w + F::MEM_WORDS);
        j.z.to_raw_words(w + 2 * F::MEM_WORDS);
        memcpy(out, w, sizeof w);
    }
};
struct msm_pending_t {
    const void* planes = nullptr;
    int nplanes = 0;
    int tail_windows = 0, nbits = 0;
    int c = 0, m = 0;
    bool folded = false;
    int ninst = 0;
    bool lazy = false;
    int pos(int idx) const {
        const int tw = idx / nbits, j = idx % nbits;
        if (ninst) return (tw & 1) * m + j;
        return folded ? c * (tw >> 1) + (tw & 1) * m + j : c * tw + j;
    }
};
template <class F>
static constexpr size_t msm_point_bytes() {
    return sizeof(F) == sizeof(fq_t) && sizeof(xyzz_mem_t<fqz_t>) > sizeof(xyzz_mem_t<F>) ? sizeof(xyzz_mem_t<fqz_t>) : sizeof(xyzz_mem_t<F>);
}
template <class F>
static xyzz_t<F> msm_plane(const msm_pending_t& pd, int i) {
    if constexpr (sizeof(F) == sizeof(fq_t)) {
        if (pd.lazy) {
            const xyzz_t<fqz_t> z = load_xyzz<fqz_t>(&((const xyzz_mem_t<fqz_t>*)pd.planes)[i]);
            if (z.is_inf()) return xyzz_t<F>::inf();
            return {z.x.to_exact(), z.y.to_exact(), z.zz.to_exact(), z.zzz.to_exact()};
        }
    }
    return load_xyzz<F>(&((const xyzz_mem_t<F>*)pd.planes)[i]);
}
template <class F>
static void msm_collect(msm_accum_t<F>& acc, const msm_pending_t& pd) {
    for (int i = 0; i < pd.nplanes; i++) acc.add(pd.pos(i), msm_plane<F>(pd, i));
}
template <class F>
static void msm_collect_inst(msm_accum_t<F>& acc, const msm_pending_t& pd, int inst) {
    const int per = 2 * pd.nbits;
    for (int i = inst * per; i < (inst + 1) * per; i++) acc.add(pd.pos(i), msm_plane<F>(pd, i));
}
struct msm_multi_t {
    const msm_inst_t* d_inst = nullptr;
    uint32_t K = 0;
    size_t npad = 0;
    size_t hn = 0;
    size_t plane_capacity = 0;
};

static size_t msm_acc_lds() {
    const long env = tuning().acc_lds;
    return env < 0 ? 0 : (size_t)env;
}
template <class F>
static bool msm_lazy_on() {
    return sizeof(F) == sizeof(fq_t) ? tuning().lazy != 0 : tuning().lazy2 != 0;
}
template <class F>
static bool msm_lazy_tail_on() {
    return sizeof(F) == sizeof(fq_t) && msm_lazy_on<F>() && tuning().lazy_tail != 0;
}
template <class F>
static size_t msm_partial_bytes() {
    return msm_lazy_tail_on<F>() ? sizeof(xyzz_mem_t<fqz_t>) : sizeof(xyzz_mem_t<F>);
}
struct msm_tail_geom_t {
    int fold_m, fold_hb, tail_windows, nbits;
    bool fold;
};
static msm_tail_geom_t msm_tail_geometry(const msm_plan_t& pl, uint32_t nwin, msm_pending_t& pd, int ninst) {
    msm_tail_geom_t g;
    const int K = pl.c - 1;
    g.fold_m = (K + 1) / 2;
    g.fold_hb = K - g.fold_m;
    g.fold = K >= 11 || (K >= 4 && pl.c * pl.W < 128);
    g.tail_windows = g.fold ? 2 * (int)nwin : (int)nwin;
    g.nbits = g.fold ? g.fold_m + 1 : pl.c;
    pd.tail_windows = g.tail_windows;
    pd.nbits = g.nbits;
    pd.nplanes = g.tail_windows * g.nbits;
    pd.c = pl.c;
    pd.m = g.fold_m;
    pd.folded = g.fold;
    pd.ninst = ninst;
    if ((!ninst && pd.nplanes > MSM_MAX_POS) || pl.c * (pl.W - 1) + (g.fold ? g.fold_m : 0) + g.nbits > MSM_MAX_POS)
        throw hip_failure{hipErrorInvalidValue, "msm: window geometry exceeds the tail's bit-position range", __LINE__};
    return g;
}
template <class F>
static void msm_tail_launch(lane_t& c, const msm_plan_t& pl, const msm_tail_geom_t& g, uint32_t nwin, uint32_t nbt, const xyzz_mem_t<F>* sums,
                            const uint32_t* start, const uint32_t* cnt, const msm_pending_t& pd, void* host_planes) {
    hipStream_t st = c.stream;
    c.planes.ensure((size_t)pd.nplanes * sizeof(xyzz_mem_t<F>));
    const bool is_g2 = sizeof(F) == sizeof(fq2_t);
    const int hex = (is_g2 && tuning().hex2) ? 1 : 0;
    int quads_planes = (tuning().tail_quads >> (is_g2 ? 0 : 2)) & 1, quads_fold = (tuning().tail_quads >> (is_g2 ? 1 : 3)) & 1;
    if (g.fold_m > 8) quads_planes = 0;
    uint32_t* fold_flags = nullptr;
    uint32_t* plane_flags = nullptr;
    if (is_g2) {
        const size_t nslots = g.fold ? ((size_t)nwin << (g.fold_m + 1)) : 0;
        c.tail_flags.ensure((nslots + (size_t)pd.nplanes) * 4);
        fold_flags = c.tail_flags.as<uint32_t>();
        plane_flags = fold_flags + nslots;
    }
    if (g.fold) {
        c.fold_sums.ensure(((size_t)nwin << (g.fold_m + 1)) * sizeof(xyzz_mem_t<F>));
        const unsigned fold_blocks = ((1u << g.fold_m) + (1u << g.fold_hb)) * (unsigned)nwin;
        unsigned fold_threads = (nbt >= (1u << 18) || fold_blocks > 512u) ? 64u : 256u;
        if (sizeof(F) <= 64 && nbt < (1u << 18) && fold_blocks > 512u && fold_blocks <= 1024u && tuning().fold_mid == 128) fold_threads = 128u;
        if (sizeof(F) > 64 && fold_threads == 256u && fold_blocks > 256u && (tuning().fold_threads2 == 128 || tuning().fold_threads2 == 64)) fold_threads = (unsigned)tuning().fold_threads2;
        if (sizeof(F) > 64 && fold_threads == 256u && fold_blocks <= 256u && (tuning().fold_small2 == 128 || tuning().fold_small2 == 64)) fold_threads = (unsigned)tuning().fold_small2;
        if (fold_threads == 64u) quads_fold = 0;
        const dim3 fold_grid((1u << g.fold_m) + (1u << g.fold_hb), (unsigned)nwin);
        hipLaunchKernelGGL((msm_fold_kernel<F>), fold_grid, dim3(fold_threads), 0, st, sums, start, cnt, c.fold_sums.as<xyzz_mem_t<F>>(), g.fold_m, g.fold_hb, hex, quads_fold,
                           fold_flags);
        if constexpr (TAIL_FLAGGED<F>::value)
            hipLaunchKernelGGL((msm_fold_fix_kernel<F>), fold_grid, dim3(64), 0, st, sums, start, cnt, c.fold_sums.as<xyzz_mem_t<F>>(), g.fold_m, g.fold_hb,
                               (const uint32_t*)fold_flags);
        const unsigned plane_threads = quads_planes ? (g.fold_m <= 4 ? 64u : g.fold_m == 5 ? 128u : 256u) : (g.fold_m <= 6 ? 64u : g.fold_m == 7 ? 128u : 256u);
        const dim3 plane_grid((unsigned)g.nbits, (unsigned)g.tail_windows);
        hipLaunchKernelGGL((msm_bitplane_kernel<F, true>), plane_grid, dim3(plane_threads), 0, st, (const xyzz_mem_t<F>*)c.fold_sums.as<xyzz_mem_t<F>>(),
                           (const uint32_t*)nullptr, (const uint32_t*)nullptr, c.planes.as<xyzz_mem_t<F>>(), pl.nb, g.fold_m, g.fold_hb, hex, quads_planes, plane_flags);
        if constexpr (TAIL_FLAGGED<F>::value)
            hipLaunchKernelGGL((msm_bitplane_fix_kernel<F, true>), plane_grid, dim3(64), 0, st, (const xyzz_mem_t<F>*)c.fold_sums.as<xyzz_mem_t<F>>(), (const uint32_t*)nullptr,
                               (const uint32_t*)nullptr, c.planes.as<xyzz_mem_t<F>>(), pl.nb, g.fold_m, g.fold_hb, (const uint32_t*)plane_flags);
    } else {
        const dim3 plane_grid((unsigned)g.nbits, (unsigned)g.tail_windows);
        hipLaunchKernelGGL((msm_bitplane_kernel<F, false>), plane_grid, dim3(256), 0, st, sums, start, cnt, c.planes.as<xyzz_mem_t<F>>(), pl.nb, 0, 0, hex, 0, plane_flags);
        if constexpr (TAIL_FLAGGED<F>::value)
            hipLaunchKernelGGL((msm_bitplane_fix_kernel<F, false>), plane_grid, dim3(64), 0, st, sums, start, cnt, c.planes.as<xyzz_mem_t<F>>(), pl.nb, 0, 0,
                               (const uint32_t*)plane_flags);
    }
    HIP_TRY(hipGetLastError());
    HIP_TRY(hipMemcpyAsync(host_planes, c.planes.p, (size_t)pd.nplanes * sizeof(xyzz_mem_t<F>), hipMemcpyDeviceToHost, st));
}
struct msm_bucket_sink_t {
    void* acc = nullptr;
    uint32_t L = 1, slot = 0, nbt = 0;
    hipEvent_t after = nullptr, done = nullptr;
};
static int msm_trace_level() {
    static const int level = getenv("SNARKVM_HIP_TRACE") ? atoi(getenv("SNARKVM_HIP_TRACE")) : 0;
    return level;
}
struct msm_phases_t {
    lane_t& c;
    bool profile;
    int trace;
    size_t n;
    const char* cur = "";
    void begin(const char* name) {
        cur = name;
        if (trace >= 2) fprintf(stderr, "[snarkvm_hip] msm n=%zu: %s ...\n", n, name);
        if (profile) c.phase_begin(name);
    }
    void end() {
        if (profile) c.phase_end();
        if (trace >= 2) {
            const hipError_t e = hipStreamSynchronize(c.stream);
            fprintf(stderr, "[snarkvm_hip] msm n=%zu: %s done (%s)\n", n, cur, hipGetErrorString(e));
        }
    }
};
template <class T>
static void msm_reduce_and_tail(lane_t& c, const msm_plan_t& pl, const msm_tail_geom_t& tg, uint32_t nwin, uint32_t nbt, int rounds, size_t T0_max, size_t T1_max,
                                const msm_bucket_sink_t* sink, msm_pending_t& pd, void* host_planes, msm_phases_t& ph) {
    hipStream_t st = c.stream;
    ph.begin("msm_reduce_partials");
    uint32_t *cnt_in = c.cnt_a.as<uint32_t>(), *cnt_out = c.cnt_b.as<uint32_t>();
    uint32_t *start_in = c.start_a.as<uint32_t>(), *start_out = c.start_b.as<uint32_t>();
    xyzz_mem_t<T> *pin = c.part_a.as<xyzz_mem_t<T>>(), *pout = c.part_b.as<xyzz_mem_t<T>>();
    size_t T_in_max = T0_max;
    for (int r = 0; r < rounds; r++) {
        size_t T_out_max = T_in_max / pl.S2 + nbt + 1;
        if (T_out_max > T1_max) T_out_max = T1_max;
        hipLaunchKernelGGL(msm_alloc_kernel, dim3((nbt + 1 + 255) / 256), dim3(256), 0, st, cnt_in, cnt_out, nbt, pl.S2);
        exclusive_scan_u32(st, cnt_out, start_out, (size_t)nbt + 1, c.scan_tmp.as<uint32_t>());
        hipLaunchKernelGGL((msm_reduce_kernel<T>), dim3((unsigned)((T_out_max + 255) / 256)), dim3(256), 0, st, pin, start_in, cnt_in, start_out, pout, nbt,
                           pl.S2);
        std::swap(cnt_in, cnt_out);
        std::swap(start_in, start_out);
        std::swap(pin, pout);
        T_in_max = T_out_max;
    }
    ph.end();
    if (sink) {
        ph.begin("msm_bucket_merge");
        if (sink->after) HIP_TRY(hipStreamWaitEvent(st, sink->after, 0));
        hipLaunchKernelGGL((msm_bucket_merge_kernel<T>), dim3((nbt + 255) / 256), dim3(256), 0, st, (const xyzz_mem_t<T>*)pin, (const uint32_t*)start_in,
                           (const uint32_t*)cnt_in, (xyzz_mem_t<T>*)sink->acc, nbt, sink->L, sink->slot);
        if (sink->done) HIP_TRY(hipEventRecord(sink->done, st));
        ph.end();
        HIP_TRY(hipGetLastError());
        pd.nplanes = 0;
        return;
    }
    ph.begin("msm_bucket_reduce");
    msm_tail_launch<T>(c, pl, tg, nwin, nbt, pin, start_in, cnt_in, pd, host_planes);
    ph.end();
}
template <class F>
static void msm_launch_accumulate(lane_t& c, const msm_plan_t& pl, const aff_mem_t<F>* vbase, uint32_t* boffp, uint32_t nbt, size_t nthreads, bool one_wave,
                                  bool ltail) {
    hipStream_t st = c.stream;
#ifdef SV_BENCH
    static const uint32_t dbg_mask = getenv("SNARKVM_HIP_DEBUG_IDX_MASK") ? (uint32_t)strtoul(getenv("SNARKVM_HIP_DEBUG_IDX_MASK"), nullptr, 0) : 0xffffffffu;
#else
    constexpr uint32_t dbg_mask = 0xffffffffu;
#endif
    const size_t tmax = nthreads + nbt + 1;
    if constexpr (sizeof(F) == sizeof(fq_t)) {
        if (msm_lazy_on<F>()) {
            if (!ltail) c.part_raw.ensure(tmax * sizeof(g1_lazy_partial_t));
            g1_lazy_partial_t* raw_out = ltail ? c.part_a.as<g1_lazy_partial_t>() : c.part_raw.as<g1_lazy_partial_t>();
            hipLaunchKernelGGL((msm_accumulate_lazy_kernel<true>), dim3((unsigned)((nthreads + 255) / 256)), dim3(256), one_wave || tuning().acc_one_wg ? msm_acc_lds() : 0, st,
                               vbase, c.sorted.as<uint32_t>(), boffp, c.start_a.as<uint32_t>(), raw_out, nbt, pl.S, dbg_mask);
            if (!ltail)
                hipLaunchKernelGGL(g1_partials_to_exact_kernel, dim3((unsigned)((tmax + 255) / 256)), dim3(256), 0, st, (const g1_lazy_partial_t*)raw_out,
                                   c.part_a.as<g1_xyzz_mem_t>(), (const uint32_t*)c.start_a.as<uint32_t>(), nbt);
            return;
        }
    } else {
#ifndef SV_NO_G2
        if (msm_lazy_on<F>()) {
            c.part_raw.ensure(tmax * sizeof(g2_pair_partial_t));
            hipLaunchKernelGGL((msm_accumulate_pair2_kernel<false>), dim3((unsigned)((2 * nthreads + 255) / 256)), dim3(256), 0, st, vbase, c.sorted.as<uint32_t>(),
                               boffp, c.start_a.as<uint32_t>(), c.part_raw.as<g2_pair_partial_t>(), nbt, pl.S, dbg_mask);
            hipLaunchKernelGGL(g2_pair_partials_to_exact_kernel, dim3((unsigned)((8 * tmax + 255) / 256)), dim3(256), 0, st,
                               (const g2_pair_partial_t*)c.part_raw.as<g2_pair_partial_t>(), c.part_a.as<xyzz_mem_t<fq2_t>>(),
                               (const uint32_t*)c.start_a.as<uint32_t>(), nbt);
            return;
        }
#endif
    }
    if (one_wave)
        hipLaunchKernelGGL((msm_accumulate_seg_kernel<F, 1, true>), dim3((unsigned)((nthreads + 255) / 256)), dim3(256), 0, st, vbase, c.sorted.as<uint32_t>(), boffp,
                           c.start_a.as<uint32_t>(), c.part_a.as<xyzz_mem_t<F>>(), nbt, pl.S, dbg_mask);
    else
        hipLaunchKernelGGL((msm_accumulate_seg_kernel<F, 1, false>), dim3((unsigned)((nthreads + 255) / 256)), dim3(256), 0, st, vbase, c.sorted.as<uint32_t>(), boffp,
                           c.start_a.as<uint32_t>(), c.part_a.as<xyzz_mem_t<F>>(), nbt, pl.S, dbg_mask);
}
template <class F>
static size_t msm_plane_bytes() {
    return (size_t)MSM_MAX_POS * msm_point_bytes<F>();
}
template <class F>
struct msm_job_t {
    const aff_mem_t<F>* bases = nullptr;
    const aff_mem_t<F>* bases1 = nullptr;
    size_t n0 = 0;
    int tables = 1;
    size_t table_stride = 0;
    int table_bits = 0;
    const uint4* scalars = nullptr;
    size_t n = 0;
    int scalars_montgomery = 0;
    int window_bits = 0;
    void* host_planes = nullptr;
    bool profile = true;
    const msm_multi_t* multi = nullptr;
    const msm_bucket_sink_t* sink = nullptr;
    hipEvent_t scalars_read = nullptr;
};
template <class F>
struct msm_layout_t {
    msm_plan_t pl;
    bool wide;
    bool fused;
    bool ltail;
    bool single_round, prefetch_ok;
    uint32_t nwin, nbt;
    size_t E_max, T0_max, T1_max;
    const aff_mem_t<F>* vbase;
    msm_tail_geom_t tg;
    msm_radix_params_t rp;
    msm_digit_params_t dp;
    int LBL;
    uint32_t B1, nbins, nseg_last;
    size_t ncounts1, tiles1, tiles2_max;
};
template <class F>
static msm_layout_t<F> msm_layout(lane_t& c, const msm_job_t<F>& j, msm_pending_t& pd) {
    const msm_multi_t* mu = j.multi;
    const size_t n = j.n;
    size_t n0 = j.bases1 ? j.n0 : n;
    if (n0 > n) n0 = n;
    msm_layout_t<F> L{};
    if (n >= ((size_t)1 << 31)) throw hip_failure{hipErrorInvalidValue, "msm: npoints must be < 2^31", __LINE__};
    const msm_plan_t pl = L.pl = msm_make_plan(n, mu ? j.table_bits : j.window_bits, j.tables, j.table_bits);
    L.wide = pl.c > 16;
    if (mu && (L.wide || pl.W != 1 || pl.c < 12 || (size_t)pl.J * mu->hn >= ((size_t)1 << 31) || n != mu->npad || n % SORT_TILE))
        throw hip_failure{hipErrorInvalidValue, "msm: geometry not eligible for a fused multi-instance run", __LINE__};
    if ((size_t)pl.Wd * n >= ((size_t)1 << 32)) throw hip_failure{hipErrorInvalidValue, "msm: windows * npoints must be < 2^32", __LINE__};
    if ((size_t)pl.J * n >= ((size_t)1 << 31)) throw hip_failure{hipErrorInvalidValue, "msm: tables * npoints must be < 2^31", __LINE__};
    const aff_mem_t<F>* vb1 = j.bases1 ? j.bases1 : j.bases;
    L.vbase = mu ? j.bases : (vb1 < j.bases ? vb1 : j.bases);
    if (!mu) {
        const size_t top0 = (size_t)(j.bases - L.vbase) + n0, top1 = (size_t)(vb1 - L.vbase) + (n - n0);
        if ((size_t)(pl.J - 1) * j.table_stride + (top0 > top1 ? top0 : top1) >= ((size_t)1 << 31))
            throw hip_failure{hipErrorInvalidValue, "msm: base slots must be addressable in 31 bits (tables * registered points < 2^31)", __LINE__};
    }
    const size_t E_max = L.E_max = (size_t)pl.Wd * n;
    const uint32_t nwin = L.nwin = mu ? mu->K : (uint32_t)pl.W;
    const uint32_t nbt = L.nbt = nwin * pl.nb;

    c.scan_tmp.ensure((scan_tmp_elems((size_t)nbt + 1)) * 4);
    c.boff.ensure(((size_t)nbt + 2) * 4);
    c.cnt_a.ensure(((size_t)nbt + 1) * 4);
    c.cnt_b.ensure(((size_t)nbt + 1) * 4);
    c.start_a.ensure(((size_t)nbt + 1) * 4);
    c.start_b.ensure(((size_t)nbt + 1) * 4);
    const size_t slack = (size_t)nbt / 32 + 64;
    L.T0_max = E_max / pl.S + nbt + 1 + slack;
    L.T1_max = L.T0_max / pl.S2 + nbt + 1 + slack;
    pd.lazy = L.ltail = msm_lazy_tail_on<F>();
    c.part_a.ensure(L.T0_max * msm_partial_bytes<F>());
    c.part_b.ensure(L.T1_max * msm_partial_bytes<F>());
    L.tg = msm_tail_geometry(pl, nwin, pd, mu ? (int)mu->K : 0);
    if (mu && (size_t)pd.nplanes > mu->plane_capacity) throw hip_failure{hipErrorInvalidValue, "msm: plane staging of the fused group too small", __LINE__};
    if (j.sink && (mu || j.sink->nbt != nbt)) throw hip_failure{hipErrorInvalidValue, "msm: bucket sink does not match the plan", __LINE__};
    c.planes.ensure((size_t)pd.nplanes * msm_partial_bytes<F>());

    L.fused = !mu && L.wide && tuning().fused && pl.c <= 22 && pl.Wd <= FUSED_MAX_ROWS;
    memcpy(L.dp.bias, pl.bias, sizeof L.dp.bias);
    L.dp.c = pl.c;
    L.dp.W = pl.Wd;
    L.dp.n = n;
    L.dp.montgomery = j.scalars_montgomery;
    L.single_round = mu || (size_t)pl.Wd * n <= ((size_t)1 << 22);
    L.prefetch_ok = (size_t)pl.Wd * n <= ((size_t)1 << 22);

    msm_radix_params_t& rp = L.rp;
    rp.n = n;
    rp.c = pl.c;
    rp.W = pl.W;
    rp.J = pl.J;
    if (mu) {
        rp.inst = mu->d_inst;
        rp.ninst = mu->K;
        rp.vstride = (uint32_t)mu->hn;
    } else {
        rp.vn0 = (uint32_t)n0;
        rp.vr0 = (uint32_t)(j.bases - L.vbase);
        rp.vr1 = (uint32_t)(vb1 - L.vbase);
        rp.vstride = (uint32_t)j.table_stride;
    }
    const int K = pl.c - 1;
    L.LBL = K < 7 ? K : 7;
    rp.LB = L.wide ? 14 : L.LBL;
    rp.HB = K - rp.LB;
    rp.nb = pl.nb;
    rp.xcd = (uint32_t)tuning().xcd;
    rp.tiles_per_row = L.fused ? (uint32_t)((n + FUSED_TILE - 1) / FUSED_TILE) : (uint32_t)((n + SORT_TILE - 1) / SORT_TILE);
    rp.TPW = (uint32_t)pl.J * rp.tiles_per_row;
    L.B1 = 1u << rp.HB;
    L.nbins = nwin * L.B1;
    L.ncounts1 = (size_t)(mu ? L.B1 : L.nbins) * rp.TPW;
    L.tiles1 = (size_t)(mu ? 1 : pl.W) * rp.TPW;
    L.nseg_last = L.wide ? L.nbins << 7 : L.nbins;
    L.tiles2_max = E_max / SORT_TILE + L.nseg_last + 1;
    return L;
}
template <class F>
static void msm_stage_digits(lane_t& c, const msm_layout_t<F>& L, const msm_job_t<F>& j, msm_phases_t& ph) {
    hipStream_t st = c.stream;
    ph.begin("msm_digits");
    c.digits.ensure(L.E_max * (L.wide ? sizeof(uint32_t) : sizeof(uint16_t)));
    size_t blocks = (j.n + 255) / 256;
    if (j.multi) {
        hipLaunchKernelGGL(msm_digits_multi_kernel, dim3((unsigned)blocks), dim3(256), 0, st, j.multi->d_inst, j.multi->K, c.digits.as<uint16_t>(), L.dp);
    } else {
        if (blocks > 256 * 16) blocks = 256 * 16;
        if (L.wide)
            hipLaunchKernelGGL((msm_digits_kernel<uint32_t>), dim3((unsigned)blocks), dim3(256), 0, st, j.scalars, c.digits.as<uint32_t>(), L.dp);
        else
            hipLaunchKernelGGL((msm_digits_kernel<uint16_t>), dim3((unsigned)blocks), dim3(256), 0, st, j.scalars, c.digits.as<uint16_t>(), L.dp);
    }
    ph.end();
    if (j.scalars_read) HIP_TRY(hipEventRecord(j.scalars_read, st));
}
template <class Fn>
static void msm_fused_width(int c, Fn&& fn) {
    switch (c) {
        case 17: return fn(std::integral_constant<int, 17>{});
        case 18: return fn(std::integral_constant<int, 18>{});
        case 19: return fn(std::integral_constant<int, 19>{});
        case 20: return fn(std::integral_constant<int, 20>{});
        case 21: return fn(std::integral_constant<int, 21>{});
        case 22: return fn(std::integral_constant<int, 22>{});
    }
}
template <class F>
static void msm_stage_level1_fused(lane_t& c, const msm_layout_t<F>& L, const msm_job_t<F>& j, msm_phases_t& ph) {
    hipStream_t st = c.stream;
    const msm_plan_t& pl = L.pl;
    const uint32_t ntiles = L.rp.tiles_per_row, keys = (uint32_t)pl.Wd * L.B1;
    const uint32_t nchunks = (ntiles + FUSED_CHUNK - 1) / FUSED_CHUNK;
    const size_t ngroups = (size_t)keys * nchunks;
    c.counts.ensure((size_t)ntiles * keys * 4);
    c.offsets.ensure((size_t)ntiles * keys * 4);
    c.fchunk.ensure(2 * ngroups * 4);
    c.scan_tmp.ensure(scan_tmp_elems(ngroups > (size_t)L.nbt + 2 ? ngroups : (size_t)L.nbt + 2) * 4);
    uint32_t* counts1 = c.counts.as<uint32_t>();
    uint32_t* off1 = c.offsets.as<uint32_t>();
    uint32_t* csum = c.fchunk.as<uint32_t>();
    uint32_t* choff = csum + ngroups;
    ph.begin("msm_scalar_read");
    const size_t hist_lds = (size_t)keys * 4;
    msm_fused_width(pl.c, [&](auto cb) {
        hipLaunchKernelGGL((radix_hist1_wide_kernel<decltype(cb)::value>), dim3(ntiles), dim3(HISTW_THREADS), hist_lds * HISTW_COPIES, st, j.scalars, counts1, L.rp, L.dp);
    });
    ph.end();
    ph.begin("msm_sort_level1");
    const unsigned key_blocks = (keys + FUSED_THREADS - 1) / FUSED_THREADS;
    hipLaunchKernelGGL(fused_chunk_sums_kernel, dim3(nchunks, key_blocks), dim3(FUSED_THREADS), 0, st, (const uint32_t*)counts1, csum, ntiles, nchunks, keys, L.B1,
                       (uint32_t)pl.W, (uint32_t)pl.J);
    exclusive_scan_u32(st, csum, choff, ngroups, c.scan_tmp.as<uint32_t>());
    hipLaunchKernelGGL(fused_tile_offsets_kernel, dim3(nchunks, key_blocks), dim3(FUSED_THREADS), 0, st, (const uint32_t*)counts1, (const uint32_t*)choff,
                       (const uint32_t*)csum, off1, c.rbinstart.as<uint32_t>(), ntiles, nchunks, keys, L.B1, (uint32_t)pl.W, (uint32_t)pl.J);
    msm_fused_width(pl.c, [&](auto cb) {
        hipLaunchKernelGGL((radix_scatter1_fused_kernel<decltype(cb)::value>), dim3(ntiles), dim3(FUSED_THREADS), 0, st, j.scalars, (const uint32_t*)counts1,
                           (const uint32_t*)off1, c.rv1.as<uint32_t>(), c.rl1.as<uint16_t>(), L.rp, L.dp);
    });
    if (j.scalars_read) HIP_TRY(hipEventRecord(j.scalars_read, st));
    ph.end();
}
template <class F>
static void msm_stage_level1(lane_t& c, const msm_layout_t<F>& L, const msm_job_t<F>& j, msm_phases_t& ph) {
    hipStream_t st = c.stream;
    c.counts.ensure(L.ncounts1 * 4);
    c.offsets.ensure(L.ncounts1 * 4);
    c.scan_tmp.ensure(scan_tmp_elems(L.ncounts1 > (size_t)L.nbt + 2 ? L.ncounts1 : (size_t)L.nbt + 2) * 4);
    c.rv1.ensure(L.E_max * 4);
    c.rl1.ensure(L.E_max * (L.wide ? 2 : 1));
    c.rcounts2.ensure(L.tiles2_max * 128 * 4);
    c.roff2.ensure(L.tiles2_max * 128 * 4);
    c.rbinstart.ensure(((size_t)L.nbins + 2) * 4);
    c.rntiles.ensure(((size_t)L.nseg_last + 2) * 4);
    c.rtstart.ensure(((size_t)L.nseg_last + 2) * 4);
    c.rbsize.ensure(((size_t)L.nbt + 3) * 4);
    c.sorted.ensure(L.E_max * 4);
    if (L.fused) return msm_stage_level1_fused(c, L, j, ph);
    uint32_t* counts1 = c.counts.as<uint32_t>();
    uint32_t* off1 = c.offsets.as<uint32_t>();
    ph.begin("msm_sort_level1");
    if (L.wide) {
        hipLaunchKernelGGL((radix_hist1_kernel<uint32_t>), dim3((unsigned)L.tiles1), dim3(SORT_THREADS), 0, st, c.digits.as<uint32_t>(), counts1, L.rp);
        exclusive_scan_u32(st, counts1, off1, L.ncounts1, c.scan_tmp.as<uint32_t>());
        hipLaunchKernelGGL((radix_scatter1_kernel<uint32_t, uint16_t>), dim3((unsigned)L.tiles1), dim3(SORT_THREADS), 0, st, c.digits.as<uint32_t>(),
                           counts1, off1, c.rv1.as<uint32_t>(), c.rl1.as<uint16_t>(), L.rp);
    } else {
        hipLaunchKernelGGL((radix_hist1_kernel<uint16_t>), dim3((unsigned)L.tiles1), dim3(SORT_THREADS), 0, st, c.digits.as<uint16_t>(), counts1, L.rp);
        exclusive_scan_u32(st, counts1, off1, L.ncounts1, c.scan_tmp.as<uint32_t>());
        hipLaunchKernelGGL((radix_scatter1_kernel<uint16_t, uint8_t>), dim3((unsigned)L.tiles1), dim3(SORT_THREADS), 0, st, c.digits.as<uint16_t>(),
                           counts1, off1, c.rv1.as<uint32_t>(), c.rl1.as<uint8_t>(), L.rp);
    }
    if (j.multi)
        hipLaunchKernelGGL(radix_bin_layout_multi_kernel, dim3((L.nbins + 1 + 255) / 256), dim3(256), 0, st, off1, counts1, L.ncounts1,
                           c.rbinstart.as<uint32_t>(), L.nbins, L.rp);
    else
        hipLaunchKernelGGL(radix_bin_layout_kernel, dim3((L.nbins + 1 + 255) / 256), dim3(256), 0, st, off1, counts1, L.ncounts1, c.rbinstart.as<uint32_t>(),
                           L.nbins, L.rp.TPW);
    ph.end();
}
static void msm_tile_segments(lane_t& c, const uint32_t* seg_start, uint32_t nseg) {
    hipLaunchKernelGGL(radix_bin_tiles_kernel, dim3((nseg + 1 + 255) / 256), dim3(256), 0, c.stream, seg_start, c.rntiles.as<uint32_t>(), nseg);
    exclusive_scan_u32(c.stream, c.rntiles.as<uint32_t>(), c.rtstart.as<uint32_t>(), (size_t)nseg + 1, c.scan_tmp.as<uint32_t>());
}
static void msm_colscan(lane_t& c, uint32_t* sizes, uint32_t nsegs, int bits, uint32_t* dmax) {
    if (nsegs <= 4096)
        hipLaunchKernelGGL(radix_colscan2_seg_kernel, dim3(nsegs), dim3(1024), 0, c.stream, c.rcounts2.as<uint32_t>(), c.roff2.as<uint32_t>(),
                           c.rtstart.as<uint32_t>(), sizes, nsegs, bits, dmax);
    else
        hipLaunchKernelGGL(radix_colscan2_kernel, dim3(((nsegs << bits) + 1 + 255) / 256), dim3(256), 0, c.stream, c.rcounts2.as<uint32_t>(),
                           c.roff2.as<uint32_t>(), c.rtstart.as<uint32_t>(), sizes, nsegs, bits, dmax);
}
template <class F>
static void msm_stage_sort_rest(lane_t& c, const msm_layout_t<F>& L, msm_phases_t& ph) {
    hipStream_t st = c.stream;
    const size_t E_max = L.E_max;
    const uint32_t nbt = L.nbt;
    uint32_t* bsize = c.rbsize.as<uint32_t>();
    uint32_t* d_max = bsize + nbt + 1;
    uint32_t* boffp = c.boff.as<uint32_t>();
    const uint32_t* seg_start = c.rbinstart.as<uint32_t>();
    uint32_t nseg = L.nbins;
    const uint32_t* v_in = c.rv1.as<uint32_t>();
    if (L.wide) {
        ph.begin("msm_sort_level2");
        const uint32_t ngroups = nseg << 7;
        const size_t tmax = E_max / SORT_TILE + nseg + 1;
        c.rv2.ensure(E_max * 4);
        c.rl2.ensure(E_max);
        c.rmid_size.ensure(((size_t)ngroups + 3) * 4);
        c.rmid_boff.ensure(((size_t)ngroups + 3) * 4);
        c.scan_tmp.ensure(scan_tmp_elems((size_t)ngroups + 2) * 4);
        uint32_t* msize = c.rmid_size.as<uint32_t>();
        uint32_t* mboff = c.rmid_boff.as<uint32_t>();
        msm_tile_segments(c, seg_start, nseg);
        hipLaunchKernelGGL((radix_hist2_kernel<uint16_t>), dim3((unsigned)tmax), dim3(SORT_THREADS), 0, st, c.rl1.as<uint16_t>(), seg_start,
                           c.rtstart.as<uint32_t>(), c.rcounts2.as<uint32_t>(), nseg, 7, 7);
        HIP_TRY(hipMemsetAsync(msize + ngroups + 1, 0, 4, st));
        msm_colscan(c, msize, nseg, 7, msize + ngroups + 1);
        exclusive_scan_u32(st, msize, mboff, (size_t)ngroups + 1, c.scan_tmp.as<uint32_t>());
        hipLaunchKernelGGL((radix_scatter2_kernel<uint16_t, uint8_t>), dim3((unsigned)tmax), dim3(SORT_THREADS), 0, st, v_in, c.rl1.as<uint16_t>(),
                           seg_start, c.rtstart.as<uint32_t>(), c.rcounts2.as<uint32_t>(), c.roff2.as<uint32_t>(), mboff, c.rv2.as<uint32_t>(),
                           c.rl2.as<uint8_t>(), nseg, 7, 7, (uint32_t)tuning().xcd);
        ph.end();
        seg_start = mboff;
        nseg = ngroups;
        v_in = c.rv2.as<uint32_t>();
    }
    ph.begin(L.wide ? "msm_sort_level3" : "msm_sort_level2");
    msm_tile_segments(c, seg_start, nseg);
    const uint8_t* rem_last = L.wide ? c.rl2.as<uint8_t>() : c.rl1.as<uint8_t>();
    hipLaunchKernelGGL((radix_hist2_kernel<uint8_t>), dim3((unsigned)L.tiles2_max), dim3(SORT_THREADS), 0, st, rem_last, seg_start,
                       c.rtstart.as<uint32_t>(), c.rcounts2.as<uint32_t>(), nseg, L.LBL, 0);
    HIP_TRY(hipMemsetAsync(d_max, 0, 4, st));
    msm_colscan(c, bsize, nseg, L.LBL, d_max);
    exclusive_scan_u32(st, bsize, boffp, (size_t)nbt + 1, c.scan_tmp.as<uint32_t>());
    hipLaunchKernelGGL((radix_scatter2_kernel<uint8_t, uint8_t>), dim3((unsigned)L.tiles2_max), dim3(SORT_THREADS), 0, st, v_in, rem_last, seg_start,
                       c.rtstart.as<uint32_t>(), c.rcounts2.as<uint32_t>(), c.roff2.as<uint32_t>(), boffp, c.sorted.as<uint32_t>(),
                       (uint8_t*)nullptr, nseg, L.LBL, 0, (uint32_t)tuning().xcd);
    ph.end();
}
template <class F>
static int msm_stage_accumulate(lane_t& c, const msm_layout_t<F>& L, const msm_job_t<F>& j, msm_phases_t& ph) {
    hipStream_t st = c.stream;
    const msm_multi_t* mu = j.multi;
    const uint32_t nbt = L.nbt;
    uint32_t* boffp = c.boff.as<uint32_t>();
    int rounds = 0;
    ph.begin("msm_accumulate");
    const int env_rounds = tuning().reduce_rounds;
    if (!L.single_round) rounds = env_rounds < 0 ? 0 : (env_rounds > 8 ? 8 : env_rounds);
    if (mu && tuning().fuse_reduce > 0) rounds = tuning().fuse_reduce > 4 ? 4 : tuning().fuse_reduce;
    if (mu && tuning().fuse_reduce < 0) rounds = mu->K >= 8 ? 1 : 0;
    hipLaunchKernelGGL(msm_alloc_seg_kernel, dim3((nbt + 1 + 255) / 256), dim3(256), 0, st, boffp, c.cnt_a.as<uint32_t>(), nbt, L.pl.S);
    exclusive_scan_u32(st, c.cnt_a.as<uint32_t>(), c.start_a.as<uint32_t>(), (size_t)nbt + 1, c.scan_tmp.as<uint32_t>());
    msm_launch_accumulate<F>(c, L.pl, L.vbase, boffp, nbt, (L.E_max + L.pl.S - 1) / L.pl.S, L.single_round && L.prefetch_ok, L.ltail);
    ph.end();
    return rounds;
}
template <class T>
struct msm_field_tag {
    using type = T;
};
template <class F, class Fn>
static void msm_on_tail_field(bool lazy, Fn&& fn) {
    if constexpr (sizeof(F) == sizeof(fq_t)) {
        if (lazy) return fn(msm_field_tag<fqz_t>{});
    }
    fn(msm_field_tag<F>{});
}
template <class F>
static msm_pending_t msm_run(lane_t& c, const msm_job_t<F>& j) {
    msm_pending_t pd;
    pd.planes = j.host_planes;
    if (j.n == 0) return pd;
    msm_phases_t ph{c, j.profile, msm_trace_level(), j.n};
    const msm_layout_t<F> L = msm_layout(c, j, pd);
    if (!L.fused) msm_stage_digits(c, L, j, ph);
    msm_stage_level1(c, L, j, ph);
    msm_stage_sort_rest(c, L, ph);
    const int rounds = msm_stage_accumulate(c, L, j, ph);
    msm_on_tail_field<F>(L.ltail, [&](auto t) {
        msm_reduce_and_tail<typename decltype(t)::type>(c, L.pl, L.tg, L.nwin, L.nbt, rounds, L.T0_max, L.T1_max, j.sink, pd, j.host_planes, ph);
    });
    return pd;
}
template <class F>
static msm_pending_t msm_tail_from_sink(lane_t& c, const msm_job_t<F>& j, const msm_bucket_sink_t& sink) {
    msm_pending_t pd;
    pd.planes = j.host_planes;
    const msm_plan_t pl = msm_make_plan(j.n, j.window_bits, j.tables, j.table_bits);
    const uint32_t nwin = (uint32_t)pl.W, nbt = nwin * pl.nb;
    if (nbt != sink.nbt) throw hip_failure{hipErrorInvalidValue, "msm: bucket sink does not match the plan", __LINE__};
    const msm_tail_geom_t tg = msm_tail_geometry(pl, nwin, pd, 0);
    c.start_a.ensure(((size_t)nbt + 1) * 4);
    c.cnt_a.ensure(((size_t)nbt + 1) * 4);
    hipLaunchKernelGGL(msm_sink_lists_kernel, dim3((nbt + 1 + 255) / 256), dim3(256), 0, c.stream, c.start_a.as<uint32_t>(), c.cnt_a.as<uint32_t>(), nbt, sink.L);
    pd.lazy = msm_lazy_tail_on<F>();
    c.phase_begin("msm_bucket_reduce");
    msm_on_tail_field<F>(pd.lazy, [&](auto t) {
        using T = typename decltype(t)::type;
        msm_tail_launch<T>(c, pl, tg, nwin, nbt, (const xyzz_mem_t<T>*)sink.acc, c.start_a.as<uint32_t>(), c.cnt_a.as<uint32_t>(), pd, j.host_planes);
    });
    c.phase_end();
    return pd;
}
template <class F>
static void msm_run_sync(lane_t& c, const msm_job_t<F>& j, void* out) {
    if (c.in_scope && c.pin_used) scope_flush();
    c.pin.ensure(msm_plane_bytes<F>());
    msm_job_t<F> staged = j;
    staged.host_planes = c.pin.p;
    const msm_pending_t pd = msm_run<F>(c, staged);
    HIP_TRY(hipStreamSynchronize(c.stream));
    const double t0 = host_now_ms();
    msm_accum_t<F>* acc = new msm_accum_t<F>();
    std::unique_ptr<msm_accum_t<F>> hold(acc);
    msm_collect<F>(*acc, pd);
    acc->finish(out);
    c.phase_host("msm_host_finish", host_now_ms() - t0);
}

template <class F>
static void convert_bases(lane_t& c, const uint8_t* d_in, size_t stride, size_t n, aff_mem_t<F>* d_out, hipStream_t st = nullptr, bool for_msm = false) {
    if (!n) return;
    const int form406 = for_msm && msm_lazy_on<F>() ? 1 : 0;
    hipLaunchKernelGGL((convert_bases_kernel<F>), dim3((unsigned)((n + 255) / 256)), dim3(256), 0, st ? st : c.stream, d_in, stride, n, d_out, form406);
    HIP_TRY(hipGetLastError());
}
static void bases_to_lazy_form(lane_t& c, g1_aff_mem_t* d, size_t slots) {
    if (!slots || !msm_lazy_on<fq_t>()) return;
    hipLaunchKernelGGL(g1_bases_to_form406_kernel, dim3((unsigned)((slots + 255) / 256)), dim3(256), 0, c.stream, d, slots);
    HIP_TRY(hipGetLastError());
}
#ifndef SV_NO_G2
static void bases_to_lazy_form(lane_t& c, aff_mem_t<fq2_t>* d, size_t slots) {
    if (!slots || !msm_lazy_on<fq2_t>()) return;
    hipLaunchKernelGGL(g2_bases_to_form406_kernel, dim3((unsigned)((slots + 255) / 256)), dim3(256), 0, c.stream, d, slots);
    HIP_TRY(hipGetLastError());
}
#endif

template <class F>
static void precompute_tables_run(lane_t& c, aff_mem_t<F>* d, size_t n, int tables, int table_bits) {
    if (tables <= 1 || !n) return;
    int run = (int)(n >> 16);
    run = run < 1 ? 1 : (run > PRE_RUN ? PRE_RUN : run);
    const size_t slab = n < PRE_SLAB ? n : PRE_SLAB;
    c.gen_pts.ensure(4 * slab * sizeof(typename F::mem_t));
    for (int j = 1; j < tables; j++)
        for (size_t lo = 0; lo < n; lo += PRE_SLAB) {
            const size_t cnt = n - lo < PRE_SLAB ? n - lo : PRE_SLAB;
            const size_t threads = (cnt + run - 1) / run;
            hipLaunchKernelGGL((precompute_table_kernel<F>), dim3((unsigned)((threads + 255) / 256)), dim3(256), 0, c.stream, d + (size_t)(j - 1) * n + lo,
                               d + (size_t)j * n + lo, cnt, table_bits, run, (typename F::mem_t*)c.gen_pts.p);
        }
    HIP_TRY(hipGetLastError());
}
```

### snarkvm_amd/csrc/runtime.hip.h

```cpp
#pragma once
#include <hip/hip_runtime.h>
#include <stdint.h>
#include <stdio.h>
#include <stdlib.h>
#include <string.h>
#include <time.h>

#include <atomic>
#include <chrono>
#include <condition_variable>
#include <deque>
#include <functional>
#include <exception>
#include <memory>
#include <mutex>
#include <stdexcept>
#include <string>
#include <thread>
#include <type_traits>
#include <utility>
#include <vector>

#include "../../include/snarkvm_hip.h"
#include "ff.hip.h"
#include "ntt.hip.h"

using namespace sv;

static RustError ok() { return RustError{0, nullptr}; }
static RustError fail(int code, const std::string& msg) {
    char* m = (char*)malloc(msg.size() + 1);
    if (m) memcpy(m, msg.c_str(), msg.size() + 1);
    return RustError{code ? code : 1, m};
}
struct hip_failure {
    hipError_t e;
    const char* what;
    int line;
};
#define HIP_TRY(x)                                             \
    do {                                                       \
        hipError_t _e = (x);                                   \
        if (_e != hipSuccess) throw hip_failure{_e, #x, __LINE__}; \
    } while (0)
static RustError from_failure(const hip_failure& f) {
    char buf[512];
    snprintf(buf, sizeof buf, "snarkvm_hip: %s failed at api.hip:%d: %s", f.what, f.line, hipGetErrorString(f.e));
    return fail((int)f.e, buf);
}

static double host_now_ms() {
    timespec ts;
    clock_gettime(CLOCK_MONOTONIC, &ts);
    return ts.tv_sec * 1e3 + ts.tv_nsec * 1e-6;
}

void sv_alloc_note(int slot, size_t bytes, double ms);
void sv_defer_free(void* p);
void sv_drain_frees();
struct alloc_timer_t {
    double t0;
    int slot;
    size_t bytes;
    alloc_timer_t(int s, size_t b) : t0(host_now_ms()), slot(s), bytes(b) {}
    ~alloc_timer_t() { sv_alloc_note(slot, bytes, host_now_ms() - t0); }
};
struct dev_buf {
    void* p = nullptr;
    size_t cap = 0;
    void ensure(size_t bytes) {
        if (bytes <= cap) return;
        size_t want = bytes + bytes / 8 + 256;
        alloc_timer_t timer(0, want);
        if (p) sv_defer_free(p);
        p = nullptr;
        cap = 0;
        if (hipMalloc(&p, want) != hipSuccess) {
            (void)hipGetLastError();
            p = nullptr;
            sv_drain_frees();
            const hipError_t e = hipMalloc(&p, want);
            if (e != hipSuccess) {
                (void)hipGetLastError();
                p = nullptr;
                throw hip_failure{e, "hipMalloc", __LINE__};
            }
        }
        cap = want;
    }
    template <class T>
    T* as() const {
        return (T*)p;
    }
};
struct pinned_buf {
    void* p = nullptr;
    size_t cap = 0;
    void ensure(size_t bytes) {
        if (bytes <= cap) return;
        size_t want = bytes + bytes / 8 + 4096;
        alloc_timer_t timer(2, want);
        if (p) HIP_TRY(hipHostFree(p));
        p = nullptr;
        cap = 0;
        HIP_TRY(hipHostMalloc(&p, want, hipHostMallocDefault));
        cap = want;
    }
    template <class T>
    T* as() const {
        return (T*)p;
    }
};

struct phase_rec {
    const char* name;
    hipEvent_t e0, e1;
    double ms;
};
struct device_t;

struct lane_t {
    device_t* dev = nullptr;
    int index = 0;
    hipStream_t stream = nullptr;
    dev_buf scalars, digits, counts, offsets, scan_tmp, sorted, boff, cnt_a, cnt_b, start_a, start_b, part_a, part_b, part_raw, planes;
    dev_buf rv1, rl1, rcounts2, roff2, rbinstart, rntiles, rtstart, rbsize;
    dev_buf rv2, rl2, rmid_size, rmid_boff;
    dev_buf fold_sums;
    dev_buf tail_flags;
    dev_buf sink_acc;
    dev_buf fchunk;
    dev_buf bases_tmp, scalars_tmp, gen_pts, gen_prod;
    dev_buf ntt_data, ntt_scratch, ntt_acc, ntt_alt;
    dev_buf serde_status;
    dev_buf poly[5];
    pinned_buf pin, pin2;
    hipStream_t alt = nullptr;
    hipEvent_t ev[4] = {};
    std::vector<void*> tw_leases;
    bool in_scope = false;
    struct deferred_out_t {
        void* dst;
        size_t off, bytes;
    };
    std::vector<deferred_out_t> deferred;
    size_t deferred_bytes = 0;
    size_t pin_used = 0;
    std::vector<hipEvent_t> scope_events;
    size_t scope_events_used = 0;
    hipEvent_t scope_event() {
        if (scope_events_used == scope_events.size()) {
            hipEvent_t e;
            HIP_TRY(hipEventCreateWithFlags(&e, hipEventDisableTiming));
            scope_events.push_back(e);
        }
        return scope_events[scope_events_used++];
    }
    std::vector<phase_rec> phases;
    std::vector<hipEvent_t> event_pool;
    size_t events_used = 0;

    hipEvent_t new_event() {
        if (events_used == event_pool.size()) {
            hipEvent_t e;
            HIP_TRY(hipEventCreate(&e));
            event_pool.push_back(e);
        }
        return event_pool[events_used++];
    }
    inline ntt_ctx_t ntt_ctx(hipStream_t st = nullptr);
    inline void begin_call();
    inline void phase_begin(const char* name);
    inline void phase_end();
    inline void phase_host(const char* name, double ms);
    inline void end_call();
    void sync_or_defer() {
        if (!in_scope) HIP_TRY(hipStreamSynchronize(stream));
    }
    void host_result(void* dst, const void* d_src, size_t bytes, bool may_defer = true) {
        if (!in_scope || !may_defer) {
            HIP_TRY(hipMemcpyAsync(dst, d_src, bytes, hipMemcpyDeviceToHost, stream));
            return;
        }
        if (deferred_bytes + bytes > pin2.cap) {
            if (!deferred.empty()) flush_scope();
            pin2.ensure(deferred_bytes + bytes > (size_t)1 << 16 ? deferred_bytes + bytes : (size_t)1 << 16);
        }
        HIP_TRY(hipMemcpyAsync(pin2.as<uint8_t>() + deferred_bytes, d_src, bytes, hipMemcpyDeviceToHost, stream));
        deferred.push_back({dst, deferred_bytes, bytes});
        deferred_bytes += (bytes + 15) & ~(size_t)15;
    }
    inline void flush_scope();
};

struct device_t {
    int logical = 0, physical = 0;
    bool ready = false;
    std::mutex init_mu;
    ntt_tables_t tb{};
    dev_buf tables_mem;
    ntt_tw_cache_t tw;
    static constexpr int LANES = 16;
    lane_t lane[LANES];
    std::mutex mu;
    std::condition_variable cv;
    uint32_t busy = 0;
    static constexpr int SCOPE_LANES_MAX = LANES - 4;
    int scope_held = 0;

    void init() {
        std::lock_guard<std::mutex> lk(init_mu);
        if (ready) return;
        for (int l = 0; l < LANES; l++) {
            lane[l].dev = this;
            lane[l].index = l;
            HIP_TRY(hipStreamCreateWithFlags(&lane[l].stream, hipStreamNonBlocking));
            HIP_TRY(hipStreamCreateWithFlags(&lane[l].alt, hipStreamNonBlocking));
            for (auto& e : lane[l].ev) HIP_TRY(hipEventCreateWithFlags(&e, hipEventDisableTiming));
        }
        static_assert(NTT_LG_MAX + 1 <= 32, "size_inv");
        const size_t entries = 8 * NTT_TW_SIZE + 2 * NTT_LOCAL + 4 * NTT_TOP + 32 + 8;
        tables_mem.ensure(entries * sizeof(fr_mem_t));
        fr_mem_t* base = tables_mem.as<fr_mem_t>();
        size_t off = 0;
        auto take = [&](size_t n) {
            fr_mem_t* r = base + off;
            off += n;
            return r;
        };
        for (int d = 0; d < 2; d++) {
            tb.pow_lo[d] = take(NTT_TW_SIZE);
            tb.pow_hi[d] = take(NTT_TW_SIZE);
            tb.g_lo[d] = take(NTT_TW_SIZE);
            tb.g_hi[d] = take(NTT_TW_SIZE);
            tb.local[d] = take(NTT_LOCAL);
            tb.pow_top[d] = take(NTT_TOP);
            tb.g_top[d] = take(NTT_TOP);
        }
        tb.size_inv = take(32);
        tb.consts = take(8);
        hipStream_t st = lane[0].stream;
        hipLaunchKernelGGL(ntt_setup_consts, dim3(1), dim3(64), 0, st, tb);
        hipLaunchKernelGGL(ntt_fill_tables, dim3(NTT_TW_SIZE / 256), dim3(256), 0, st, tb);
        HIP_TRY(hipGetLastError());
        HIP_TRY(hipStreamSynchronize(st));
        ready = true;
    }
    int take(lane_t** out, int want) {
        std::unique_lock<std::mutex> lk(mu);
        cv.wait(lk, [&] { return busy != (1u << LANES) - 1; });
        int got = 0;
        for (int l = 0; l < LANES && got < want; l++)
            if (!(busy & (1u << l))) {
                busy |= 1u << l;
                out[got++] = &lane[l];
            }
        return got;
    }
    bool try_take(lane_t** out) {
        std::lock_guard<std::mutex> lk(mu);
        for (int l = 0; l < LANES; l++)
            if (!(busy & (1u << l))) {
                busy |= 1u << l;
                *out = &lane[l];
                return true;
            }
        return false;
    }
    int try_take_n(lane_t** out, int want) {
        std::lock_guard<std::mutex> lk(mu);
        int got = 0;
        for (int l = 0; l < LANES && got < want; l++)
            if (!(busy & (1u << l))) {
                busy |= 1u << l;
                out[got++] = &lane[l];
            }
        return got;
    }
    lane_t* take_for_scope(bool block) {
        std::unique_lock<std::mutex> lk(mu);
        auto room = [&] { return busy != (1u << LANES) - 1 && scope_held < SCOPE_LANES_MAX; };
        if (block)
            cv.wait(lk, room);
        else if (!room())
            return nullptr;
        for (int i = 0; i < LANES; i++) {
            const int l = block ? i : LANES - 1 - i;
            if (!(busy & (1u << l))) {
                busy |= 1u << l;
                scope_held++;
                return &lane[l];
            }
        }
        return nullptr;
    }
    void give(lane_t* l, bool from_scope = false) {
        {
            std::lock_guard<std::mutex> lk(mu);
            busy &= ~(1u << l->index);
            if (from_scope) scope_held--;
        }
        cv.notify_all();
    }
};

struct runtime_t {
    std::mutex cfg_mu;
    std::vector<int> want;
    std::vector<std::unique_ptr<device_t>> devs;
    bool configured = false;
    std::atomic<uint32_t> rr{0};
    std::atomic<bool> profiling{false};
    std::mutex prof_mu;
    std::vector<std::pair<std::string, double>> last_phases;

    void configure() {
        std::lock_guard<std::mutex> lk(cfg_mu);
        if (configured) return;
        int ndev = 0;
        hipError_t e = hipGetDeviceCount(&ndev);
        if (e != hipSuccess || ndev == 0) throw hip_failure{e == hipSuccess ? hipErrorNoDevice : e, "hipGetDeviceCount (no MI355X visible)", __LINE__};
        std::vector<int> ids = want;
        if (ids.empty()) {
            if (const char* env = getenv("SNARKVM_HIP_DEVICES")) {
                for (const char* p = env; *p;) {
                    char* end = nullptr;
                    long v = strtol(p, &end, 10);
                    if (end == p) break;
                    ids.push_back((int)v);
                    p = (*end == ',') ? end + 1 : end;
                }
            }
        }
        if (ids.empty())
            for (int d = 0; d < ndev; d++) ids.push_back(d);
        for (int id : ids)
            if (id < 0 || id >= ndev) throw hip_failure{hipErrorInvalidDevice, "device index out of range (snarkvm_hip_set_devices / SNARKVM_HIP_DEVICES)", __LINE__};
        for (size_t i = 0; i < ids.size(); i++) {
            devs.emplace_back(new device_t());
            devs.back()->logical = (int)i;
            devs.back()->physical = ids[i];
        }
        configured = true;
    }
    int ndev() {
        configure();
        return (int)devs.size();
    }
    int device_of(const void* ptr) {
        configure();
        hipPointerAttribute_t at;
        if (!ptr || hipPointerGetAttributes(&at, ptr) != hipSuccess) {
            (void)hipGetLastError();
            return -1;
        }
        std::vector<int> match;
        for (auto& d : devs)
            if (d->physical == at.device) match.push_back(d->logical);
        if (match.empty()) return -1;
        return match[rr.fetch_add(1) % match.size()];
    }
};
extern runtime_t g_rt;

static void tu_set_kernel_attributes();
static void tu_kernel_attributes(int logical) {
    static std::mutex mu;
    static std::vector<char> done;
    std::lock_guard<std::mutex> lk(mu);
    if ((int)done.size() <= logical) done.resize(logical + 1, 0);
    if (done[logical]) return;
    tu_set_kernel_attributes();
    done[logical] = 1;
}

static constexpr int SCOPE_AUX_MAX = 7;
struct scope_pending_t {
    hipEvent_t done;
    std::function<void()> finish;
    const void* tag;
};
struct thread_scope_t {
    lane_t* lane = nullptr;
    int prev_device = -1;
    unsigned flags = 0;
    lane_t* aux[SCOPE_AUX_MAX] = {};
    int naux = 0;
    unsigned aux_rr = 0;
    bool aux_exhausted = false;
    std::vector<scope_pending_t> pending;
    thread_scope_t() = default;
    thread_scope_t(const thread_scope_t&) = default;
    thread_scope_t& operator=(const thread_scope_t&) = default;
    ~thread_scope_t();
};
extern thread_local thread_scope_t g_tl_scope;
static thread_scope_t& tl_scope() { return g_tl_scope; }
static void scope_flush() {
    thread_scope_t& sc = tl_scope();
    if (!sc.lane) return;
    std::exception_ptr err;
    for (scope_pending_t& p : sc.pending) {
        try {
            HIP_TRY(hipEventSynchronize(p.done));
            p.finish();
        } catch (...) {
            if (!err) err = std::current_exception();
        }
    }
    sc.pending.clear();
    try {
        sc.lane->flush_scope();
        for (int i = 0; i < sc.naux; i++) HIP_TRY(hipStreamSynchronize(sc.aux[i]->stream));
    } catch (...) {
        if (!err) err = std::current_exception();
    }
    sc.lane->pin_used = 0;
    sc.lane->scope_events_used = 0;
    for (int i = 0; i < sc.naux; i++) sc.aux[i]->pin_used = 0, sc.aux[i]->scope_events_used = 0;
    if (err) std::rethrow_exception(err);
}
static void scope_collect(const void* tag) {
    thread_scope_t& sc = tl_scope();
    if (!sc.lane) return;
    std::exception_ptr err;
    if (tag) {
        auto ready = [](const scope_pending_t& p) {
            const hipError_t e = hipEventQuery(p.done);
            if (e == hipSuccess) return true;
            (void)hipGetLastError();
            return false;
        };
        auto wanted_ready = [&]() {
            for (const scope_pending_t& p : sc.pending)
                if (p.tag == tag && !ready(p)) return false;
            return true;
        };
        for (size_t i = 0; i < sc.pending.size() && !wanted_ready();) {
            if (sc.pending[i].tag != tag && ready(sc.pending[i])) {
                try {
                    sc.pending[i].finish();
                } catch (...) {
                    if (!err) err = std::current_exception();
                }
                sc.pending.erase(sc.pending.begin() + (ptrdiff_t)i);
            } else {
                i++;
            }
        }
    }
    std::vector<scope_pending_t> keep;
    for (scope_pending_t& p : sc.pending) {
        if (tag && p.tag != tag) {
            keep.push_back(std::move(p));
            continue;
        }
        try {
            HIP_TRY(hipEventSynchronize(p.done));
            p.finish();
        } catch (...) {
            if (!err) err = std::current_exception();
        }
    }
    sc.pending.swap(keep);
    if (sc.pending.empty()) {
        sc.lane->pin_used = 0, sc.lane->scope_events_used = 0;
        for (int i = 0; i < sc.naux; i++) sc.aux[i]->pin_used = 0, sc.aux[i]->scope_events_used = 0;
    }
    if (err) std::rethrow_exception(err);
}
struct lane_guard {
    std::vector<lane_t*> lanes;
    int prev_device = -1;
    bool borrowed = false;
    bool first_borrowed = false;
    lane_guard() {}
    lane_guard(const lane_guard&) = delete;
    explicit lane_guard(int dev) {
        lane_t* sl = tl_scope().lane;
        if (sl && (dev < 0 || (dev < (int)g_rt.devs.size() && g_rt.devs[dev]->physical == sl->dev->physical))) {
            borrowed = true;
            lanes.push_back(sl);
            tu_kernel_attributes(sl->dev->logical);
            return;
        }
        acquire(dev, 1);
    }
    void acquire(int dev, int want) {
        scope_flush();
        g_rt.configure();
        const int nd = (int)g_rt.devs.size();
        if (dev >= nd) throw hip_failure{hipErrorInvalidDevice, "logical device index out of range", __LINE__};
        if (lane_t* sl = tl_scope().lane) {
            if (dev < 0 || g_rt.devs[dev]->physical == sl->dev->physical) {
                lanes.push_back(sl);
                first_borrowed = true;
                tu_kernel_attributes(sl->dev->logical);
                lane_t* more[device_t::LANES];
                const int n = want > 1 ? sl->dev->try_take_n(more, want - 1) : 0;
                for (int i = 0; i < n; i++) lanes.push_back(more[i]);
                return;
            }
        }
        if (prev_device < 0 && hipGetDevice(&prev_device) != hipSuccess) prev_device = 0;
        device_t* d = nullptr;
        lane_t* got[device_t::LANES];
        int n = 0;
        if (dev >= 0) {
            d = g_rt.devs[dev].get();
        } else {
            const uint32_t s = g_rt.rr.fetch_add(1);
            for (int i = 0; i < nd && !d; i++) {
                device_t* cand = g_rt.devs[(s + i) % nd].get();
                if (want == 1) {
                    if (cand->try_take(&got[0])) {
                        d = cand;
                        n = 1;
                    }
                } else {
                    d = cand;
                }
            }
            if (!d) d = g_rt.devs[s % nd].get();
        }
        if (!n) n = d->take(got, want);
        try {
            HIP_TRY(hipSetDevice(d->physical));
            d->init();
            tu_kernel_attributes(d->logical);
        } catch (...) {
            for (int i = 0; i < n; i++) d->give(got[i]);
            if (prev_device >= 0) (void)hipSetDevice(prev_device);
            throw;
        }
        for (int i = 0; i < n; i++) lanes.push_back(got[i]);
    }
    lane_t& c() { return *lanes[0]; }
    ~lane_guard() {
        if (borrowed) return;
        for (size_t i = first_borrowed ? 1 : 0; i < lanes.size(); i++) lanes[i]->dev->give(lanes[i]);
        if (prev_device >= 0) (void)hipSetDevice(prev_device);
    }
};

inline ntt_ctx_t lane_t::ntt_ctx(hipStream_t st) { return ntt_ctx_t{st ? st : stream, &dev->tb, &dev->tw, &tw_leases}; }
inline void lane_t::begin_call() {
    phases.clear();
    events_used = 0;
}
inline void lane_t::phase_begin(const char* name) {
    if (!g_rt.profiling.load(std::memory_order_relaxed)) return;
    phase_rec r{name, new_event(), new_event(), 0.0};
    HIP_TRY(hipEventRecord(r.e0, stream));
    phases.push_back(r);
}
inline void lane_t::phase_end() {
    if (!g_rt.profiling.load(std::memory_order_relaxed) || phases.empty()) return;
    HIP_TRY(hipEventRecord(phases.back().e1, stream));
}
inline void lane_t::phase_host(const char* name, double ms) {
    if (!g_rt.profiling.load(std::memory_order_relaxed)) return;
    phases.push_back(phase_rec{name, nullptr, nullptr, ms});
}
static void ntt_tw_release(device_t* dev, std::vector<void*>& leases) { ntt_tw_release_entries(dev->tw, leases); }
inline void lane_t::flush_scope() {
    HIP_TRY(hipStreamSynchronize(stream));
    for (const deferred_out_t& d : deferred) memcpy(d.dst, pin2.as<uint8_t>() + d.off, d.bytes);
    deferred.clear();
    deferred_bytes = 0;
    if (!tw_leases.empty()) ntt_tw_release(dev, tw_leases);
    sv_drain_frees();
}
inline void lane_t::end_call() {
    if (in_scope) return;
    sv_drain_frees();
    if (!tw_leases.empty()) {
        HIP_TRY(hipStreamSynchronize(stream));
        ntt_tw_release(dev, tw_leases);
    }
    if (phases.empty()) return;
    HIP_TRY(hipStreamSynchronize(stream));
    std::vector<std::pair<std::string, double>> out;
    for (auto& r : phases) {
        if (r.e0) {
            float ms = 0;
            HIP_TRY(hipEventElapsedTime(&ms, r.e0, r.e1));
            r.ms = ms;
        }
        out.emplace_back(r.name, r.ms);
    }
    std::lock_guard<std::mutex> lk(g_rt.prof_mu);
    g_rt.last_phases.swap(out);
}

template <class Fn>
static void for_each_device(const std::vector<int>& devices, Fn fn) {
    if (devices.size() <= 1) {
        for (int d : devices) fn(d);
        return;
    }
    std::vector<std::thread> th;
    std::vector<std::exception_ptr> errs(devices.size());
    for (size_t i = 0; i < devices.size(); i++)
        th.emplace_back([&, i] {
            try {
                fn(devices[i]);
            } catch (...) {
                errs[i] = std::current_exception();
            }
        });
    for (auto& t : th) t.join();
    for (auto& e : errs)
        if (e) std::rethrow_exception(e);
}

template <class Fn>
static void host_parallel_for(size_t n, int max_threads, Fn fn) {
    size_t T = n / 4;
    if (T > (size_t)max_threads) T = (size_t)max_threads;
    if (T <= 1) {
        for (size_t i = 0; i < n; i++) fn(i);
        return;
    }
    std::atomic<size_t> next{0};
    std::vector<std::exception_ptr> errs(T);
    auto work = [&](size_t t) {
        try {
            for (size_t i; (i = next.fetch_add(1)) < n;) fn(i);
        } catch (...) {
            errs[t] = std::current_exception();
        }
    };
    std::vector<std::thread> th;
    for (size_t t = 1; t < T; t++) th.emplace_back(work, t);
    work(0);
    for (auto& x : th) x.join();
    for (auto& e : errs)
        if (e) std::rethrow_exception(e);
}

#define API_BEGIN_DEV(devsel)                      \
    try {                                          \
        lane_guard _lg(devsel);                    \
        lane_t& c = _lg.c();                       \
        c.begin_call();
#define API_BEGIN API_BEGIN_DEV(-1)
#define API_TRY try {
#define API_CATCH                                  \
    return ok();                                   \
    }                                              \
    catch (const hip_failure& f) {                 \
        return from_failure(f);                    \
    }                                              \
    catch (const std::exception& e) {              \
        return fail(1, std::string("snarkvm_hip: ") + e.what()); \
    }                                              \
    catch (...) {                                  \
        return fail(1, "snarkvm_hip: unknown error"); \
    }
#define API_END   \
    c.end_call(); \
    API_CATCH
static int device_for(const void* ptr, int on_device) {
    if (!on_device || !ptr) return -1;
    const int d = g_rt.device_of(ptr);
    if (d < 0) throw hip_failure{hipErrorInvalidValue, "device pointer does not belong to a device in use (snarkvm_hip_set_devices)", __LINE__};
    return d;
}
```

### snarkvm_amd/csrc/tuning.hip.h

```cpp
#pragma once
#include <stdio.h>
#include <stdlib.h>
#include <string.h>

namespace sv {

struct tuning_t {
    int lazy = 1, lazy2 = 1, fused = 1;
    long acc_lds = 96 * 1024;
    int acc_one_wg = 0, reduce_rounds = 1, fuse_batch = 1, fuse_max_k = 64, fuse_reduce = -1, coalesce = 1, coalesce_us = 40, lanes = 0;
    int msm_chunk_lg = 20, scalar_chunk_lg = 22, taper = 1, ring_lanes = 3, seg = 0, seg2 = 0, fold_l = 0, scan1 = 1;
    int ntt_min_tiles = 256, ntt_full_tw = 1, ntt_fold = 1, ntt_batch = 1;
    int xcd = 1, fold_threads2 = 128, coalesce_slots = 2, ramp = 3, scalar_geo = 4, lazy_tail = 1, horner2 = 1, hex2 = 1, group_quad = 1, tail_quads = 13, fold_small2 = 256, fold_mid = 128;

    bool set(const char* key, long v) {
#define SV_TUNE_KEY(name)                  \
    if (!strcmp(key, #name)) {             \
        name = (decltype(name))v;          \
        return true;                       \
    }
        SV_TUNE_KEY(lazy) SV_TUNE_KEY(lazy2) SV_TUNE_KEY(fused) SV_TUNE_KEY(acc_lds)
        SV_TUNE_KEY(acc_one_wg) SV_TUNE_KEY(reduce_rounds) SV_TUNE_KEY(fuse_batch) SV_TUNE_KEY(fuse_max_k) SV_TUNE_KEY(fuse_reduce) SV_TUNE_KEY(coalesce)
        SV_TUNE_KEY(coalesce_us) SV_TUNE_KEY(lanes) SV_TUNE_KEY(msm_chunk_lg) SV_TUNE_KEY(scalar_chunk_lg) SV_TUNE_KEY(taper) SV_TUNE_KEY(ring_lanes) SV_TUNE_KEY(seg) SV_TUNE_KEY(seg2)
        SV_TUNE_KEY(fold_l) SV_TUNE_KEY(scan1) SV_TUNE_KEY(ntt_min_tiles) SV_TUNE_KEY(ntt_full_tw) SV_TUNE_KEY(ntt_fold)
        SV_TUNE_KEY(ntt_batch) SV_TUNE_KEY(xcd) SV_TUNE_KEY(fold_threads2) SV_TUNE_KEY(coalesce_slots) SV_TUNE_KEY(ramp) SV_TUNE_KEY(scalar_geo) SV_TUNE_KEY(lazy_tail) SV_TUNE_KEY(horner2) SV_TUNE_KEY(hex2) SV_TUNE_KEY(group_quad) SV_TUNE_KEY(tail_quads) SV_TUNE_KEY(fold_small2) SV_TUNE_KEY(fold_mid)
#undef SV_TUNE_KEY
        return false;
    }
    void parse(const char* s) {
        while (s && *s) {
            while (*s == ',' || *s == ' ') s++;
            const char* eq = strchr(s, '=');
            const char* end = strchr(s, ',');
            if (!end) end = s + strlen(s);
            if (!*s) break;
            char key[32] = {0};
            if (!eq || eq > end || (size_t)(eq - s) >= sizeof key) {
                fprintf(stderr, "[snarkvm_hip] SNARKVM_HIP_TUNING: malformed item at \"%s\" (ignored)\n", s);
            } else {
                memcpy(key, s, (size_t)(eq - s));
                char* num_end = nullptr;
                const long v = strtol(eq + 1, &num_end, 0);
                if (num_end == eq + 1 || !set(key, v)) fprintf(stderr, "[snarkvm_hip] SNARKVM_HIP_TUNING: unknown key or bad value \"%s\" (ignored)\n", key);
            }
            s = end;
        }
    }
    void clamp() {
        auto fix = [](const char* key, auto& v, long lo, long hi) {
            if ((long)v < lo || (long)v > hi) {
                const long was = (long)v;
                v = (decltype(v + 0))((long)v < lo ? lo : hi);
                fprintf(stderr, "[snarkvm_hip] SNARKVM_HIP_TUNING: %s=%ld is out of range [%ld, %ld]; using %ld\n", key, was, lo, hi, (long)v);
            }
        };
        fix("coalesce_slots", coalesce_slots, 1, 8);
        fix("coalesce_us", coalesce_us, 0, 100000);
        fix("fuse_max_k", fuse_max_k, 2, 256);
        fix("fuse_reduce", fuse_reduce, -1, 4);
        fix("reduce_rounds", reduce_rounds, 0, 8);
        fix("lanes", lanes, 0, 8);
        fix("ring_lanes", ring_lanes, 2, 8);
        fix("ntt_min_tiles", ntt_min_tiles, 1, 1 << 20);
        fix("acc_lds", acc_lds, 0, 160 * 1024);
        fix("msm_chunk_lg", msm_chunk_lg, 16, 30);
        fix("scalar_chunk_lg", scalar_chunk_lg, 18, 30);
        fix("ramp", ramp, 0, 6);
        fix("scalar_geo", scalar_geo, 0, 16);
        fix("seg", seg, 0, 4096);
        fix("seg2", seg2, 0, 256);
        fix("fold_l", fold_l, 0, 64);
    }
};
inline const tuning_t& tuning() {
    static const tuning_t t = [] {
        tuning_t v;
        v.parse(getenv("SNARKVM_HIP_TUNING"));
        v.clamp();
        return v;
    }();
    return t;
}

}
```

Baseline: 578.0 million pairs/s.

## Merge bucket partial sums in place instead of the separate reduce pass

Adds an in-place merge of partial bucket sums for multi-round G1 MSMs. Light buckets are collapsed into their first slot and heavy buckets are reduced into a spare region appended to part_a. The fold kernel gains a gaps mode that reads per-bucket start/count instead of assuming contiguous layout. The aim is to avoid the ping-pong reduce rounds through part_b and their scans, at the cost of extra spare memory and several small kernels.

```diff
diff --git a/snarkvm_amd/csrc/api_g2.hip b/snarkvm_amd/csrc/api_g2.hip
--- a/snarkvm_amd/csrc/api_g2.hip
+++ b/snarkvm_amd/csrc/api_g2.hip
@@ -315,7 +315,7 @@
         uint32_t* plane_flags = fold_flags + nslots;
         const dim3 fold_grid((1u << m) + (1u << hb), 1u), plane_grid((unsigned)nbits, 2u);
         hipLaunchKernelGGL((msm_fold_kernel<fq2_t>), fold_grid, dim3((unsigned)threads), 0, c.stream, (const mem_t*)c.part_a.as<mem_t>(),
-                           (const uint32_t*)c.start_a.as<uint32_t>(), (const uint32_t*)c.cnt_a.as<uint32_t>(), out, m, hb, hex, quads & 2 ? 1 : 0, fold_flags);
+                           (const uint32_t*)c.start_a.as<uint32_t>(), (const uint32_t*)c.cnt_a.as<uint32_t>(), out, m, hb, hex, quads & 2 ? 1 : 0, 0, fold_flags);
         hipLaunchKernelGGL((msm_fold_fix_kernel<fq2_t>), fold_grid, dim3(64), 0, c.stream, (const mem_t*)c.part_a.as<mem_t>(), (const uint32_t*)c.start_a.as<uint32_t>(),
                            (const uint32_t*)c.cnt_a.as<uint32_t>(), out, m, hb, (const uint32_t*)fold_flags);
         hipLaunchKernelGGL((msm_bitplane_kernel<fq2_t, true>), plane_grid, dim3((unsigned)plane_threads), 0, c.stream, (const mem_t*)c.fold_sums.as<mem_t>(),
diff --git a/snarkvm_amd/csrc/api_tailtest.hip b/snarkvm_amd/csrc/api_tailtest.hip
--- a/snarkvm_amd/csrc/api_tailtest.hip
+++ b/snarkvm_amd/csrc/api_tailtest.hip
@@ -4,7 +4,7 @@
 
 namespace {
 
-enum { TT_REDUCE = 0, TT_MERGE, TT_FOLD, TT_SPARSE };
+enum { TT_REDUCE = 0, TT_MERGE, TT_FOLD, TT_SPARSE, TT_INPLACE, TT_INPLACE_FOLD };
 struct tt_geom_t {
     int m, hb, W, nb, S2, L, slot, fold_threads, plane_threads, hex, quads, run_fix;
 };
@@ -105,7 +105,9 @@
         }
         tt_put<T, E>(&ent[e], p);
     }
-    c.part_a.ensure((a.nentries + 1) * sizeof(mem_t));
+    const bool inplace = a.stage == TT_INPLACE || a.stage == TT_INPLACE_FOLD;
+    const size_t spare = inplace ? msm_merge_spare(a.nentries, (uint32_t)g.S2) : 0;
+    c.part_a.ensure((a.nentries + spare + 1) * sizeof(mem_t));
     c.start_a.ensure((nbt + 1) * 4);
     c.cnt_a.ensure((nbt + 1) * 4);
     if (a.nentries) HIP_TRY(hipMemcpyAsync(c.part_a.p, ent.data(), a.nentries * sizeof(mem_t), hipMemcpyHostToDevice, st));
@@ -116,7 +118,22 @@
     const uint32_t *start = c.start_a.as<uint32_t>(), *cnt = c.cnt_a.as<uint32_t>();
     std::vector<mem_t> got(a.nout);
     std::vector<uint32_t> flag_copy(a.nout, 0);
-    if (a.stage == TT_REDUCE) {
+    if (inplace) {
+        msm_plan_t pl{};
+        pl.S2 = (uint32_t)g.S2;
+        c.cnt_b.ensure((nbt + 1) * 4);
+        c.start_b.ensure((nbt + 1) * 4);
+        c.merge_heavy.ensure((nbt + 1) * 4);
+        c.scan_tmp.ensure(scan_tmp_elems(nbt + 1) * 4);
+        HIP_TRY(hipMemsetAsync(c.part_a.as<mem_t>() + a.nentries, 0xff, (spare + 1) * sizeof(mem_t), st));
+        msm_merge_partials<T>(c, pl, (uint32_t)nbt, a.nentries);
+        HIP_TRY(hipGetLastError());
+    }
+    if (a.stage == TT_INPLACE) {
+        HIP_TRY(hipMemcpyAsync(a.aux, c.start_a.p, nbt * 4, hipMemcpyDeviceToHost, st));
+        HIP_TRY(hipMemcpyAsync(a.aux + nbt, c.cnt_a.p, nbt * 4, hipMemcpyDeviceToHost, st));
+        HIP_TRY(hipMemcpyAsync(got.data(), c.part_a.p, a.nout * sizeof(mem_t), hipMemcpyDeviceToHost, st));
+    } else if (a.stage == TT_REDUCE) {
         c.cnt_b.ensure((nbt + 1) * 4);
         c.start_b.ensure((nbt + 1) * 4);
         c.scan_tmp.ensure(scan_tmp_elems(nbt + 1) * 4);
@@ -138,7 +155,7 @@
         HIP_TRY(hipGetLastError());
         HIP_TRY(hipMemcpyAsync(got.data(), c.part_b.p, nacc * sizeof(mem_t), hipMemcpyDeviceToHost, st));
     } else {
-        const bool fold = a.stage == TT_FOLD;
+        const bool fold = a.stage == TT_FOLD || a.stage == TT_INPLACE_FOLD;
         const int nbits = fold ? g.m + 1 : tt_log2((uint32_t)g.nb) + 1;
         const size_t nslots = fold ? (size_t)g.W << (g.m + 1) : 0, nplanes = (size_t)(fold ? 2 * g.W : g.W) * nbits;
         c.fold_sums.ensure((nslots + 1) * sizeof(mem_t));
@@ -154,7 +171,7 @@
         const dim3 plane_grid((unsigned)nbits, (unsigned)(fold ? 2 * g.W : g.W));
         if (fold) {
             const dim3 fold_grid((1u << g.m) + (1u << g.hb), (unsigned)g.W);
-            hipLaunchKernelGGL((msm_fold_kernel<T>), fold_grid, dim3((unsigned)g.fold_threads), 0, st, sums, start, cnt, fs, g.m, g.hb, g.hex, (g.quads >> 1) & 1, fold_flags);
+            hipLaunchKernelGGL((msm_fold_kernel<T>), fold_grid, dim3((unsigned)g.fold_threads), 0, st, sums, start, cnt, fs, g.m, g.hb, g.hex, (g.quads >> 1) & 1, inplace ? 1 : 0, fold_flags);
             if constexpr (TAIL_FLAGGED<T>::value)
                 if (g.run_fix) hipLaunchKernelGGL((msm_fold_fix_kernel<T>), fold_grid, dim3(64), 0, st, sums, start, cnt, fs, g.m, g.hb, (const uint32_t*)fold_flags);
             hipLaunchKernelGGL((msm_bitplane_kernel<T, true>), plane_grid, dim3((unsigned)g.plane_threads), 0, st, (const mem_t*)fs, (const uint32_t*)nullptr,
@@ -185,6 +202,7 @@
             continue;
         }
         a.status[i] = (a.stage == TT_MERGE && memcmp(&got[i], &ent[a.nentries + i], sizeof(mem_t)) == 0) ? 2u : 0u;
+        if (a.stage == TT_INPLACE && i < a.nentries && memcmp(&got[i], &ent[i], sizeof(mem_t)) == 0) a.status[i] = 2u;
         const jac_t<E> j = tt_get<T, E>(&got[i]).to_jacobian();
         j.x.to_raw_words(dst);
         j.y.to_raw_words(dst + CW);
@@ -200,11 +218,11 @@
                                        size_t nentries, const uint32_t* start, const uint32_t* cnt, size_t nbt, void* out, uint32_t* status, uint32_t* flags, size_t nout,
                                        uint32_t* aux) {
     API_BEGIN
-    if (arith < 0 || arith > 2 || stage < TT_REDUCE || stage > TT_SPARSE) tt_bad("devtest_msm_tail: arith must be 0 .. 2, stage 0 .. 3", __LINE__);
+    if (arith < 0 || arith > 2 || stage < TT_REDUCE || stage > TT_INPLACE_FOLD) tt_bad("devtest_msm_tail: arith must be 0 .. 2, stage 0 .. 5", __LINE__);
 #ifdef SV_NO_G2
     if (arith == 2) throw hip_failure{hipErrorNotSupported, "this development build was compiled without G2 (SV_NO_G2)", __LINE__};
 #endif
-    if (!geom || !points || !terms || !seeds || !start || !cnt || !out || !status || !flags || (stage == TT_REDUCE && !aux))
+    if (!geom || !points || !terms || !seeds || !start || !cnt || !out || !status || !flags || ((stage == TT_REDUCE || stage == TT_INPLACE) && !aux))
         tt_bad("devtest_msm_tail: null argument", __LINE__);
     tt_args_t a;
     a.stage = stage;
@@ -222,10 +240,15 @@
         for (size_t k = 0; k < nbt; k++) T += ((size_t)cnt[k] + g.S2 - 1) / g.S2;
         if (nout < T || nout > T + 4096 || nout == 0) tt_bad("devtest_msm_tail: nout must cover the round's partial sums (and at most 4096 more)", __LINE__);
         want_out = nout;
+    } else if (stage == TT_INPLACE) {
+        if (arith == 2 || g.S2 < 2 || g.S2 > 64) tt_bad("devtest_msm_tail: the in-place merge is a G1 step, S2 must be 2 .. 64", __LINE__);
+        want_out = nentries + msm_merge_spare(nentries, (uint32_t)g.S2);
+        contiguous = true;
     } else if (stage == TT_MERGE) {
         if (g.L < 1 || g.L > 8 || g.slot < 0 || g.slot >= g.L) tt_bad("devtest_msm_tail: L must be 1 .. 8, slot < L", __LINE__);
         want_out = nbt * (size_t)g.L;
-    } else if (stage == TT_FOLD) {
+    } else if (stage == TT_FOLD || stage == TT_INPLACE_FOLD) {
+        if (stage == TT_INPLACE_FOLD && (arith == 2 || g.S2 < 2 || g.S2 > 64)) tt_bad("devtest_msm_tail: the in-place merge is a G1 step, S2 must be 2 .. 64", __LINE__);
         if (g.m < 1 || g.hb < 1 || g.hb > g.m || g.hb > 11 || g.m > 11 || g.W < 1 || g.W > 64) tt_bad("devtest_msm_tail: fold geometry out of range (1 <= hb <= m <= 11)", __LINE__);
         if (!threads_ok(g.fold_threads) || !threads_ok(g.plane_threads)) tt_bad("devtest_msm_tail: threads must be 64, 128 or 256", __LINE__);
         if (((g.quads & 2) && g.fold_threads == 64) || ((g.quads & 1) && g.plane_threads == 64)) tt_bad("devtest_msm_tail: no quad-strided loop with 64 threads", __LINE__);
diff --git a/snarkvm_amd/csrc/msm.hip.h b/snarkvm_amd/csrc/msm.hip.h
--- a/snarkvm_amd/csrc/msm.hip.h
+++ b/snarkvm_amd/csrc/msm.hip.h
@@ -344,6 +344,52 @@
     store_xyzz<F>(&out[t], acc);
 }
 
+static __global__ void msm_merge_alloc_kernel(const uint32_t* __restrict__ cnt, uint32_t* __restrict__ light, uint32_t* __restrict__ heavy, uint32_t nbt, uint32_t S2) {
+    const uint32_t k = blockIdx.x * blockDim.x + threadIdx.x;
+    if (k > nbt) return;
+    const uint32_t c = k == nbt ? 0u : cnt[k];
+    light[k] = (c >= 2 && c <= S2) ? 1u : 0u;
+    heavy[k] = c > S2 ? (c + S2 - 1) / S2 : 0u;
+}
+template <class F>
+__global__ void __launch_bounds__(256) msm_merge_heavy_kernel(xyzz_mem_t<F>* __restrict__ sums, const uint32_t* __restrict__ start, const uint32_t* __restrict__ cnt,
+                                                              const uint32_t* __restrict__ hstart, uint32_t nbt, uint32_t S2, uint32_t spare) {
+    const uint32_t t = blockIdx.x * blockDim.x + threadIdx.x;
+    if (t >= hstart[nbt]) return;
+    const uint32_t k = find_bucket(hstart, nbt, t);
+    const uint32_t lo = start[k] + (t - hstart[k]) * S2;
+    uint32_t hi = lo + S2;
+    const uint32_t end = start[k] + cnt[k];
+    if (hi > end) hi = end;
+    xyzz_t<F> acc = load_xyzz<F>(&sums[lo]);
+    for (uint32_t pos = lo + 1; pos < hi; pos++) acc.add(load_xyzz<F>(&sums[pos]));
+    store_xyzz<F>(&sums[spare + t], acc);
+}
+static __global__ void msm_merge_lists_kernel(uint32_t* __restrict__ start, uint32_t* __restrict__ cnt, const uint32_t* __restrict__ lstart,
+                                              const uint32_t* __restrict__ hstart, uint32_t* __restrict__ list, uint32_t nbt, uint32_t spare) {
+    const uint32_t k = blockIdx.x * blockDim.x + threadIdx.x;
+    if (k >= nbt) return;
+    if (lstart[k + 1] != lstart[k]) list[lstart[k]] = k;
+    const uint32_t g = hstart[k + 1] - hstart[k];
+    if (g) {
+        start[k] = spare + hstart[k];
+        cnt[k] = g;
+    }
+}
+template <class F>
+__global__ void __launch_bounds__(256) msm_merge_light_kernel(xyzz_mem_t<F>* __restrict__ sums, const uint32_t* __restrict__ start, uint32_t* __restrict__ cnt,
+                                                              const uint32_t* __restrict__ list, const uint32_t* __restrict__ lstart, uint32_t nbt) {
+    const uint32_t t = blockIdx.x * blockDim.x + threadIdx.x;
+    if (t >= lstart[nbt]) return;
+    const uint32_t k = list[t];
+    const uint32_t lo = start[k], hi = lo + cnt[k];
+    xyzz_t<F> acc = load_xyzz<F>(&sums[lo]);
+    for (uint32_t pos = lo + 1; pos < hi; pos++) acc.add(load_xyzz<F>(&sums[pos]));
+    store_xyzz<F>(&sums[lo], acc);
+    cnt[k] = 1;
+}
+static inline size_t msm_merge_spare(size_t total, uint32_t S2) { return total / S2 + total / (S2 + 1) + 1; }
+
 template <class F>
 __global__ void __launch_bounds__(256) msm_bucket_merge_kernel(const xyzz_mem_t<F>* __restrict__ part, const uint32_t* __restrict__ start,
                                                                const uint32_t* __restrict__ cnt, xyzz_mem_t<F>* __restrict__ acc, uint32_t nbt, uint32_t L,
@@ -603,7 +649,7 @@
 template <class F>
 __global__ void __launch_bounds__(256, TAIL_WAVES<F>::value) msm_fold_kernel(const xyzz_mem_t<F>* __restrict__ sums, const uint32_t* __restrict__ start,
                                                        const uint32_t* __restrict__ cnt, xyzz_mem_t<F>* __restrict__ out, int m, int hb, int hex, int quads,
-                                                       uint32_t* __restrict__ flags) {
+                                                       int gaps, uint32_t* __restrict__ flags) {
     __shared__ xyzz_mem_t<F> sh[16];
     __shared__ uint32_t s_off[TAIL_MAX_SEG + 1], s_start[TAIL_MAX_SEG], s_tmp[256];
     const uint32_t nlo = 1u << m, nhi = 1u << hb;
@@ -615,16 +661,16 @@
     const size_t slot = ((size_t)w << (m + 1)) + (column ? fixed : nlo + fixed - 1);
     bool dbl = false;
     uint32_t nseg;
-    if (column) {
-        for (uint32_t i = threadIdx.x; i < nhi; i += blockDim.x) {
-            const uint32_t k = kbase + (i << m) + fixed;
+    if (column || gaps) {
+        nseg = column ? nhi : nlo;
+        for (uint32_t i = threadIdx.x; i < nseg; i += blockDim.x) {
+            const uint32_t k = column ? kbase + (i << m) + fixed : kbase + (fixed << m) + i;
             s_start[i] = start[k];
             s_off[i + 1] = cnt[k];
         }
         if (threadIdx.x == 0) s_off[0] = 0;
         __syncthreads();
-        block_running_sums(s_off, nhi, s_tmp);
-        nseg = nhi;
+        block_running_sums(s_off, nseg, s_tmp);
     } else {
         const uint32_t k0 = kbase + (fixed << m);
         if (threadIdx.x == 0) {
@@ -770,7 +816,7 @@
 }
 
 #define SV_TAIL_FOLD_KERNELS(PREFIX, F)                                                                                                                             \
-    PREFIX template __global__ void msm_fold_kernel<F>(const xyzz_mem_t<F>*, const uint32_t*, const uint32_t*, xyzz_mem_t<F>*, int, int, int, int, uint32_t*);
+    PREFIX template __global__ void msm_fold_kernel<F>(const xyzz_mem_t<F>*, const uint32_t*, const uint32_t*, xyzz_mem_t<F>*, int, int, int, int, int, uint32_t*);
 #define SV_TAIL_PLANE_KERNELS(PREFIX, F)                                                                                                                            \
     PREFIX template __global__ void msm_bitplane_kernel<F, true>(const xyzz_mem_t<F>*, const uint32_t*, const uint32_t*, xyzz_mem_t<F>*, uint32_t, int, int, int, int, uint32_t*); \
     PREFIX template __global__ void msm_bitplane_kernel<F, false>(const xyzz_mem_t<F>*, const uint32_t*, const uint32_t*, xyzz_mem_t<F>*, uint32_t, int, int, int, int, uint32_t*);
diff --git a/snarkvm_amd/csrc/msm_run.hip.h b/snarkvm_amd/csrc/msm_run.hip.h
--- a/snarkvm_amd/csrc/msm_run.hip.h
+++ b/snarkvm_amd/csrc/msm_run.hip.h
@@ -134,8 +134,9 @@
 }
 template <class F>
 static void msm_tail_launch(lane_t& c, const msm_plan_t& pl, const msm_tail_geom_t& g, uint32_t nwin, uint32_t nbt, const xyzz_mem_t<F>* sums,
-                            const uint32_t* start, const uint32_t* cnt, const msm_pending_t& pd, void* host_planes) {
-    hipStream_t st = c.stream;
+                            const uint32_t* start, const uint32_t* cnt, const msm_pending_t& pd, void* host_planes, bool gaps = false) {
+    hipStream_t st = c.stream;
+    if (gaps && !g.fold) throw hip_failure{hipErrorInvalidValue, "msm: the unfolded bit planes need the partial sums laid out bucket after bucket", __LINE__};
     c.planes.ensure((size_t)pd.nplanes * sizeof(xyzz_mem_t<F>));
     const bool is_g2 = sizeof(F) == sizeof(fq2_t);
     const int hex = (is_g2 && tuning().hex2) ? 1 : 0;
@@ -159,7 +160,7 @@
         if (fold_threads == 64u) quads_fold = 0;
         const dim3 fold_grid((1u << g.fold_m) + (1u << g.fold_hb), (unsigned)nwin);
         hipLaunchKernelGGL((msm_fold_kernel<F>), fold_grid, dim3(fold_threads), 0, st, sums, start, cnt, c.fold_sums.as<xyzz_mem_t<F>>(), g.fold_m, g.fold_hb, hex, quads_fold,
-                           fold_flags);
+                           gaps ? 1 : 0, fold_flags);
         if constexpr (TAIL_FLAGGED<F>::value)
             hipLaunchKernelGGL((msm_fold_fix_kernel<F>), fold_grid, dim3(64), 0, st, sums, start, cnt, c.fold_sums.as<xyzz_mem_t<F>>(), g.fold_m, g.fold_hb,
                                (const uint32_t*)fold_flags);
@@ -209,10 +210,56 @@
     }
 };
 template <class T>
-static void msm_reduce_and_tail(lane_t& c, const msm_plan_t& pl, const msm_tail_geom_t& tg, uint32_t nwin, uint32_t nbt, int rounds, size_t T0_max, size_t T1_max,
-                                const msm_bucket_sink_t* sink, msm_pending_t& pd, void* host_planes, msm_phases_t& ph) {
+static void msm_sink_merge(lane_t& c, const msm_bucket_sink_t* sink, const xyzz_mem_t<T>* sums, const uint32_t* start, const uint32_t* cnt, uint32_t nbt, msm_pending_t& pd,
+                           msm_phases_t& ph) {
+    hipStream_t st = c.stream;
+    ph.begin("msm_bucket_merge");
+    if (sink->after) HIP_TRY(hipStreamWaitEvent(st, sink->after, 0));
+    hipLaunchKernelGGL((msm_bucket_merge_kernel<T>), dim3((nbt + 255) / 256), dim3(256), 0, st, sums, start, cnt, (xyzz_mem_t<T>*)sink->acc, nbt, sink->L, sink->slot);
+    if (sink->done) HIP_TRY(hipEventRecord(sink->done, st));
+    ph.end();
+    HIP_TRY(hipGetLastError());
+    pd.nplanes = 0;
+}
+template <class T>
+static bool msm_merge_on(const msm_tail_geom_t& tg, bool sink, int rounds) {
+    return rounds >= 1 && tuning().tail_merge && !TAIL_FLAGGED<T>::value && (sink || tg.fold);
+}
+template <class T>
+static void msm_merge_partials(lane_t& c, const msm_plan_t& pl, uint32_t nbt, size_t T0_max) {
+    hipStream_t st = c.stream;
+    uint32_t *start = c.start_a.as<uint32_t>(), *cnt = c.cnt_a.as<uint32_t>();
+    uint32_t *lstart = c.cnt_b.as<uint32_t>(), *list = c.start_b.as<uint32_t>(), *hstart = c.merge_heavy.as<uint32_t>();
+    xyzz_mem_t<T>* sums = c.part_a.as<xyzz_mem_t<T>>();
+    const unsigned bucket_blocks = (nbt + 1 + 255) / 256;
+    hipLaunchKernelGGL(msm_merge_alloc_kernel, dim3(bucket_blocks), dim3(256), 0, st, (const uint32_t*)cnt, lstart, hstart, nbt, pl.S2);
+    exclusive_scan_u32(st, lstart, lstart, (size_t)nbt + 1, c.scan_tmp.as<uint32_t>());
+    exclusive_scan_u32(st, hstart, hstart, (size_t)nbt + 1, c.scan_tmp.as<uint32_t>());
+    const size_t heavy_max = msm_merge_spare(T0_max, pl.S2);
+    hipLaunchKernelGGL((msm_merge_heavy_kernel<T>), dim3((unsigned)((heavy_max + 255) / 256)), dim3(256), 0, st, sums, (const uint32_t*)start, (const uint32_t*)cnt,
+                       (const uint32_t*)hstart, nbt, pl.S2, (uint32_t)T0_max);
+    hipLaunchKernelGGL(msm_merge_lists_kernel, dim3(bucket_blocks), dim3(256), 0, st, start, cnt, (const uint32_t*)lstart, (const uint32_t*)hstart, list, nbt, (uint32_t)T0_max);
+    const size_t light_max = T0_max / 2 < nbt ? T0_max / 2 : nbt;
+    hipLaunchKernelGGL((msm_merge_light_kernel<T>), dim3((unsigned)((light_max + 255) / 256)), dim3(256), 0, st, sums, (const uint32_t*)start, cnt, (const uint32_t*)list,
+                       (const uint32_t*)lstart, nbt);
+}
+template <class T>
+static void msm_reduce_and_tail(lane_t& c, const msm_plan_t& pl, const msm_tail_geom_t& tg, uint32_t nwin, uint32_t nbt, int rounds, bool multi_round, size_t T0_max,
+                                size_t T1_max, const msm_bucket_sink_t* sink, msm_pending_t& pd, void* host_planes, msm_phases_t& ph) {
     hipStream_t st = c.stream;
     ph.begin("msm_reduce_partials");
+    if (multi_round && msm_merge_on<T>(tg, sink != nullptr, rounds)) {
+        msm_merge_partials<T>(c, pl, nbt, T0_max);
+        ph.end();
+        if (sink) {
+            msm_sink_merge<T>(c, sink, c.part_a.as<xyzz_mem_t<T>>(), c.start_a.as<uint32_t>(), c.cnt_a.as<uint32_t>(), nbt, pd, ph);
+            return;
+        }
+        ph.begin("msm_bucket_reduce");
+        msm_tail_launch<T>(c, pl, tg, nwin, nbt, c.part_a.as<xyzz_mem_t<T>>(), c.start_a.as<uint32_t>(), c.cnt_a.as<uint32_t>(), pd, host_planes, true);
+        ph.end();
+        return;
+    }
     uint32_t *cnt_in = c.cnt_a.as<uint32_t>(), *cnt_out = c.cnt_b.as<uint32_t>();
     uint32_t *start_in = c.start_a.as<uint32_t>(), *start_out = c.start_b.as<uint32_t>();
     xyzz_mem_t<T> *pin = c.part_a.as<xyzz_mem_t<T>>(), *pout = c.part_b.as<xyzz_mem_t<T>>();
@@ -231,14 +278,7 @@
     }
     ph.end();
     if (sink) {
-        ph.begin("msm_bucket_merge");
-        if (sink->after) HIP_TRY(hipStreamWaitEvent(st, sink->after, 0));
-        hipLaunchKernelGGL((msm_bucket_merge_kernel<T>), dim3((nbt + 255) / 256), dim3(256), 0, st, (const xyzz_mem_t<T>*)pin, (const uint32_t*)start_in,
-                           (const uint32_t*)cnt_in, (xyzz_mem_t<T>*)sink->acc, nbt, sink->L, sink->slot);
-        if (sink->done) HIP_TRY(hipEventRecord(sink->done, st));
-        ph.end();
-        HIP_TRY(hipGetLastError());
-        pd.nplanes = 0;
+        msm_sink_merge<T>(c, sink, pin, start_in, cnt_in, nbt, pd, ph);
         return;
     }
     ph.begin("msm_bucket_reduce");
@@ -360,8 +400,9 @@
     L.T0_max = E_max / pl.S + nbt + 1 + slack;
     L.T1_max = L.T0_max / pl.S2 + nbt + 1 + slack;
     pd.lazy = L.ltail = msm_lazy_tail_on<F>();
-    c.part_a.ensure(L.T0_max * msm_partial_bytes<F>());
+    c.part_a.ensure((L.T0_max + msm_merge_spare(L.T0_max, pl.S2)) * msm_partial_bytes<F>());
     c.part_b.ensure(L.T1_max * msm_partial_bytes<F>());
+    c.merge_heavy.ensure(((size_t)nbt + 1) * 4);
     L.tg = msm_tail_geometry(pl, nwin, pd, mu ? (int)mu->K : 0);
     if (mu && (size_t)pd.nplanes > mu->plane_capacity) throw hip_failure{hipErrorInvalidValue, "msm: plane staging of the fused group too small", __LINE__};
     if (j.sink && (mu || j.sink->nbt != nbt)) throw hip_failure{hipErrorInvalidValue, "msm: bucket sink does not match the plan", __LINE__};
@@ -373,7 +414,7 @@
     L.dp.W = pl.Wd;
     L.dp.n = n;
     L.dp.montgomery = j.scalars_montgomery;
-    L.single_round = mu || (size_t)pl.Wd * n <= ((size_t)1 << 22);
+    L.single_round = mu || (size_t)pl.Wd * n <= ((size_t)1 << tuning().multi_round_lg);
     L.prefetch_ok = (size_t)pl.Wd * n <= ((size_t)1 << 22);
 
     msm_radix_params_t& rp = L.rp;
@@ -611,7 +652,7 @@
     msm_stage_sort_rest(c, L, ph);
     const int rounds = msm_stage_accumulate(c, L, j, ph);
     msm_on_tail_field<F>(L.ltail, [&](auto t) {
-        msm_reduce_and_tail<typename decltype(t)::type>(c, L.pl, L.tg, L.nwin, L.nbt, rounds, L.T0_max, L.T1_max, j.sink, pd, j.host_planes, ph);
+        msm_reduce_and_tail<typename decltype(t)::type>(c, L.pl, L.tg, L.nwin, L.nbt, rounds, !L.single_round, L.T0_max, L.T1_max, j.sink, pd, j.host_planes, ph);
     });
     return pd;
 }
diff --git a/snarkvm_amd/csrc/runtime.hip.h b/snarkvm_amd/csrc/runtime.hip.h
--- a/snarkvm_amd/csrc/runtime.hip.h
+++ b/snarkvm_amd/csrc/runtime.hip.h
@@ -126,6 +126,7 @@
     dev_buf scalars, digits, counts, offsets, scan_tmp, sorted, boff, cnt_a, cnt_b, start_a, start_b, part_a, part_b, part_raw, planes;
     dev_buf rv1, rl1, rcounts2, roff2, rbinstart, rntiles, rtstart, rbsize;
     dev_buf rv2, rl2, rmid_size, rmid_boff;
+    dev_buf merge_heavy;
     dev_buf fold_sums;
     dev_buf tail_flags;
     dev_buf sink_acc;
diff --git a/snarkvm_amd/csrc/tuning.hip.h b/snarkvm_amd/csrc/tuning.hip.h
--- a/snarkvm_amd/csrc/tuning.hip.h
+++ b/snarkvm_amd/csrc/tuning.hip.h
@@ -11,7 +11,7 @@
     int acc_one_wg = 0, reduce_rounds = 1, fuse_batch = 1, fuse_max_k = 64, fuse_reduce = -1, coalesce = 1, coalesce_us = 40, lanes = 0;
     int msm_chunk_lg = 20, scalar_chunk_lg = 22, taper = 1, ring_lanes = 3, seg = 0, seg2 = 0, fold_l = 0, scan1 = 1;
     int ntt_min_tiles = 256, ntt_full_tw = 1, ntt_fold = 1, ntt_batch = 1;
-    int xcd = 1, fold_threads2 = 128, coalesce_slots = 2, ramp = 3, scalar_geo = 4, lazy_tail = 1, horner2 = 1, hex2 = 1, group_quad = 1, tail_quads = 13, fold_small2 = 256, fold_mid = 128;
+    int xcd = 1, fold_threads2 = 128, coalesce_slots = 2, ramp = 3, scalar_geo = 4, lazy_tail = 1, horner2 = 1, hex2 = 1, group_quad = 1, tail_quads = 13, fold_small2 = 256, fold_mid = 128, tail_merge = 1, multi_round_lg = 22;
 
     bool set(const char* key, long v) {
 #define SV_TUNE_KEY(name)                  \
@@ -23,7 +23,7 @@
         SV_TUNE_KEY(acc_one_wg) SV_TUNE_KEY(reduce_rounds) SV_TUNE_KEY(fuse_batch) SV_TUNE_KEY(fuse_max_k) SV_TUNE_KEY(fuse_reduce) SV_TUNE_KEY(coalesce)
         SV_TUNE_KEY(coalesce_us) SV_TUNE_KEY(lanes) SV_TUNE_KEY(msm_chunk_lg) SV_TUNE_KEY(scalar_chunk_lg) SV_TUNE_KEY(taper) SV_TUNE_KEY(ring_lanes) SV_TUNE_KEY(seg) SV_TUNE_KEY(seg2)
         SV_TUNE_KEY(fold_l) SV_TUNE_KEY(scan1) SV_TUNE_KEY(ntt_min_tiles) SV_TUNE_KEY(ntt_full_tw) SV_TUNE_KEY(ntt_fold)
-        SV_TUNE_KEY(ntt_batch) SV_TUNE_KEY(xcd) SV_TUNE_KEY(fold_threads2) SV_TUNE_KEY(coalesce_slots) SV_TUNE_KEY(ramp) SV_TUNE_KEY(scalar_geo) SV_TUNE_KEY(lazy_tail) SV_TUNE_KEY(horner2) SV_TUNE_KEY(hex2) SV_TUNE_KEY(group_quad) SV_TUNE_KEY(tail_quads) SV_TUNE_KEY(fold_small2) SV_TUNE_KEY(fold_mid)
+        SV_TUNE_KEY(ntt_batch) SV_TUNE_KEY(xcd) SV_TUNE_KEY(fold_threads2) SV_TUNE_KEY(coalesce_slots) SV_TUNE_KEY(ramp) SV_TUNE_KEY(scalar_geo) SV_TUNE_KEY(lazy_tail) SV_TUNE_KEY(horner2) SV_TUNE_KEY(hex2) SV_TUNE_KEY(group_quad) SV_TUNE_KEY(tail_quads) SV_TUNE_KEY(fold_small2) SV_TUNE_KEY(fold_mid) SV_TUNE_KEY(tail_merge) SV_TUNE_KEY(multi_round_lg)
 #undef SV_TUNE_KEY
         return false;
     }
@@ -70,6 +70,7 @@
         fix("seg", seg, 0, 4096);
         fix("seg2", seg2, 0, 256);
         fix("fold_l", fold_l, 0, 64);
+        fix("multi_round_lg", multi_round_lg, 12, 30);
     }
 };
 inline const tuning_t& tuning() {
```

Measured after the change: 578.7 million pairs/s (median of 2 runs). No clear change (+0.1%).
